# ohjay/snn-modulation-classification

Measured on AMD Instinct MI355X. Metric: IQ windows/sec (RadioML 2x128, T=128), higher is better.
Workload: dtype f32

## Files before the change

### experiments/ablate_c32d.hip

```cpp
#include "../snn_modulation_classification_amd/csrc/dcll_hip.hip"
#include <vector>
int main(int argc, char **argv)
{
    const bool presig = argc > 1 && argv[1][0] == 'p';
    const bool tp = argc > 1 && argv[1][0] == 't';
    const bool co = argc > 1 && !presig && !tp;
    const int B = 1024, T = 128;
    size_t nin = (size_t)T * B * 32 * 8;
    uint32_t *spk_in, *spk_out; float *W, *bias, *tau4, *e0, *e1, *arp, *pv; unsigned long long *dbg;
    hipMalloc(&spk_in, nin * 4); hipMalloc(&spk_out, nin * 4); hipMemset(spk_in, 0x11, nin * 4);
    hipMalloc(&W, 32 * 32 * 49 * 4); hipMalloc(&bias, 128); hipMalloc(&tau4, 512);
    std::vector<float> hw(32 * 32 * 49, 1e-6f), hb(32, 1e-4f), ht(128, 0.9f);
    hipMemcpy(W, hw.data(), hw.size() * 4, hipMemcpyHostToDevice);
    hipMemcpy(bias, hb.data(), 128, hipMemcpyHostToDevice); hipMemcpy(tau4, ht.data(), 512, hipMemcpyHostToDevice);
    size_t ns = (size_t)B * 32 * 256;
    hipMalloc(&e0, ns * 4); hipMalloc(&e1, ns * 4); hipMalloc(&arp, ns * 4);
    hipMemset(e0, 0, ns * 4); hipMemset(e1, 0, ns * 4); hipMemset(arp, 0, ns * 4);
    hipMalloc(&pv, (size_t)T * ns * 4); hipMalloc(&dbg, 4096); hipMemset(dbg, 0, 4096);
    float *dbg_v = nullptr;
    if (presig) hipMalloc(&dbg_v, (size_t)T * ns * 4);
    hipEvent_t a, b; hipEventCreate(&a); hipEventCreate(&b);
    float *pv2 = nullptr, *Wro = nullptr, *ro = nullptr;
    hipStream_t side = nullptr;
    int lo, hi;
    hipDeviceGetStreamPriorityRange(&lo, &hi);
    hipStream_t hot;
    hipStreamCreateWithPriority(&hot, hipStreamNonBlocking, hi);
    if (co) {
        hipMalloc(&pv2, (size_t)T * ns * 4); hipMemset(pv2, 0, (size_t)T * ns * 4);
        hipMalloc(&Wro, 24 * 8192 * 4); hipMemset(Wro, 0, 24 * 8192 * 4); hipMalloc(&ro, (size_t)T * B * 24 * 4);
        hipStreamCreateWithPriority(&side, hipStreamNonBlocking, lo);
    }
    auto launch_side = [&](int n) {
        for (int i = 0; i < n; ++i) dcll_launch_readout_direct(pv2, Wro, nullptr, ro, (long)T * B, 8192, 24, side);
    };
    if (tp) {
        const char *names[3] = {"k_lif_seq_c32rp (row-paired)", "k_lif_seq_c32d (time-paired)", "k_lif_seq_c32d, chain phase only"};
        for (int mode = 0; mode < 3; ++mode) {
            for (int rep = 0; rep < 3 && mode < 2; ++rep) {
                hipMemset(e0, 0, ns * 4); hipMemset(e1, 0, ns * 4); hipMemset(arp, 0, ns * 4);
                hipEventRecord(a);
                if (mode == 0)
                    hipLaunchKernelGGL((k_lif_seq_c32rp<true, 1, 0>), dim3(B), dim3(512), 0, 0, spk_in, dcll_wsrc{W, nullptr, nullptr}, bias, tau4, e0, e1, arp, spk_out, pv, (float *)nullptr, T, B, 0.65f, 1.0f);
                else
                    hipLaunchKernelGGL((k_lif_seq_c32d<true, 1, 0>), dim3(B), dim3(512), 0, 0, spk_in, dcll_wsrc{W, nullptr, nullptr}, bias, tau4, e0, e1, arp, spk_out, pv, (float *)nullptr, T, B, 0.65f, 1.0f);
                hipEventRecord(b); hipEventSynchronize(b);
                float ms; hipEventElapsedTime(&ms, a, b);
                printf("%s B=%d T=%d: %.3f ms\n", names[mode], B, T, ms);
            }
            hipMemset(dbg, 0, 4096);
            if (mode == 0)
                hipLaunchKernelGGL((k_lif_seq_c32rp<true, 1, 1>), dim3(B), dim3(512), 0, 0, spk_in, dcll_wsrc{W, nullptr, nullptr}, bias, tau4, e0, e1, arp, spk_out, pv, (float *)dbg, T, B, 0.65f, 1.0f);
            else if (mode == 1)
                hipLaunchKernelGGL((k_lif_seq_c32d<true, 1, 1>), dim3(B), dim3(512), 0, 0, spk_in, dcll_wsrc{W, nullptr, nullptr}, bias, tau4, e0, e1, arp, spk_out, pv, (float *)dbg, T, B, 0.65f, 1.0f);
            else
                hipLaunchKernelGGL((k_lif_seq_c32d<true, 1, 9>), dim3(B), dim3(512), 0, 0, spk_in, dcll_wsrc{W, nullptr, nullptr}, bias, tau4, e0, e1, arp, spk_out, pv, (float *)dbg, T, B, 0.65f, 1.0f);
            hipDeviceSynchronize();
            unsigned long long h4[64];
            hipMemcpy(h4, dbg, 512, hipMemcpyDeviceToHost);
            const double nst4 = 4.0 * T + 8;
            printf("%s: cycles per stage | non-MFMA phase | barrier 2 | chains + slot write | barrier 1\n", names[mode]);
            for (int w = 0; w < 8; ++w)
                printf("  w%d: %8.0f | %7.0f | %7.0f | %7.0f | %7.0f\n", w, h4[w * 8] / nst4, h4[w * 8 + 1] / nst4, h4[w * 8 + 2] / nst4,
                       h4[w * 8 + 3] / nst4, h4[w * 8 + 4] / nst4);
        }
        return 0;
    }
    if (presig) {
        for (int mode = 0; mode < 2; ++mode) {
            float best = 1e30f;
            for (int rep = 0; rep < 4; ++rep) {
                hipEventRecord(a);
                if (mode == 0)
                    hipLaunchKernelGGL((k_lif_seq_c32rp<true, 1, 0>), dim3(B), dim3(512), 0, 0, spk_in, dcll_wsrc{W, nullptr, nullptr}, bias, tau4, e0, e1, arp, spk_out, pv, (float *)nullptr, T, B, 0.65f, 1.0f);
                else
                    hipLaunchKernelGGL((k_lif_seq_c32rp<true, 2, 0>), dim3(B), dim3(512), 0, 0, spk_in, dcll_wsrc{W, nullptr, nullptr}, bias, tau4, e0, e1, arp, spk_out, (float *)nullptr, pv, T, B, 0.65f, 1.0f);
                hipEventRecord(b); hipEventSynchronize(b);
                float ms; hipEventElapsedTime(&ms, a, b);
                if (ms < best) best = ms;
            }
            printf("k_lif_seq_c32rp B=%d T=%d, buffer = %s: %.3f ms (best of 4)\n", B, T, mode ? "v (pv_presigmoid)" : "sigmoid(v)", best);
            if (mode == 0)
                hipLaunchKernelGGL((k_lif_seq_c32rp<true, 3, 1>), dim3(B), dim3(512), 0, 0, spk_in, dcll_wsrc{W, nullptr, nullptr}, bias, tau4, e0, e1, arp, spk_out, pv, (float *)dbg_v, T, B, 0.65f, 1.0f);
            else
                hipLaunchKernelGGL((k_lif_seq_c32rp<true, 2, 1>), dim3(B), dim3(512), 0, 0, spk_in, dcll_wsrc{W, nullptr, nullptr}, bias, tau4, e0, e1, arp, spk_out, (float *)nullptr, (float *)dbg_v, T, B, 0.65f, 1.0f);
            hipDeviceSynchronize();
            unsigned long long h3[64];
            hipMemcpy(h3, dbg_v, 512, hipMemcpyDeviceToHost);
            const double nst3 = 4.0 * T + 8;
            printf("  cycles per stage | non-MFMA phase | barrier 2 | chains + slot write | barrier 1%s\n", mode ? "" : "   (this variant also stores v: OUT = 3)");
            for (int w = 0; w < 8; ++w)
                printf("  w%d: %8.0f | %7.0f | %7.0f | %7.0f | %7.0f\n", w, h3[w * 8] / nst3, h3[w * 8 + 1] / nst3, h3[w * 8 + 2] / nst3,
                       h3[w * 8 + 3] / nst3, h3[w * 8 + 4] / nst3);
        }
        return 0;
    }
    for (int rep = 0; rep < 3 && !co; ++rep) {
        hipEventRecord(a);
        hipLaunchKernelGGL((k_lif_seq_c32rp<true, 1, 0>), dim3(B), dim3(512), 0, 0, spk_in, dcll_wsrc{W, nullptr, nullptr}, bias, tau4, e0, e1, arp, spk_out, pv, (float *)nullptr, T, B, 0.65f, 1.0f);
        hipEventRecord(b); hipEventSynchronize(b);
        float ms; hipEventElapsedTime(&ms, a, b);
        printf("k_lif_seq_c32rp B=%d T=%d: %.2f ms (ideal at 157.3 TF: %.2f)\n", B, T, ms, 2.0 * 32 * 1568 * 256 * (double)T * B / 157.3e12 * 1e3);
    }
    if (!co) {
        for (int rep = 0; rep < 3; ++rep) {
            hipEventRecord(a);
            hipLaunchKernelGGL((k_lif_seq_c32rp<true, 1, 2>), dim3(B), dim3(512), 0, 0, spk_in, dcll_wsrc{W, nullptr, nullptr}, bias, tau4, e0, e1, arp, spk_out, pv, (float *)nullptr, T, B, 0.65f, 1.0f);
            hipEventRecord(b); hipEventSynchronize(b);
            float ms; hipEventElapsedTime(&ms, a, b);
            printf("k_lif_seq_c32rp, conflict-free B reads (wrong data): %.2f ms\n", ms);
        }
        hipLaunchKernelGGL((k_lif_seq_c32rp<true, 1, 3>), dim3(B), dim3(512), 0, 0, spk_in, dcll_wsrc{W, nullptr, nullptr}, bias, tau4, e0, e1, arp, spk_out, pv, (float *)dbg, T, B, 0.65f, 1.0f);
        unsigned long long h2[64];
        hipMemcpy(h2, dbg, 512, hipMemcpyDeviceToHost);
        const double nst2 = 4.0 * T + 8;
        printf("conflict-free variant: cycles per stage | non-MFMA phase | barrier 2 | chains + slot write | barrier 1\n");
        for (int w = 0; w < 8; ++w)
            printf("  w%d: %8.0f | %7.0f | %7.0f | %7.0f | %7.0f\n", w, h2[w * 8] / nst2, h2[w * 8 + 1] / nst2, h2[w * 8 + 2] / nst2,
                   h2[w * 8 + 3] / nst2, h2[w * 8 + 4] / nst2);
        hipMemset(dbg, 0, 4096);
    }
    if (co) {
        hipDeviceSynchronize();
        launch_side(40);
        hipEventRecord(a, hot);
    }
    hipLaunchKernelGGL((k_lif_seq_c32rp<true, 1, 1>), dim3(B), dim3(512), 0, hot, spk_in, dcll_wsrc{W, nullptr, nullptr}, bias, tau4, e0, e1, arp, spk_out, pv, (float *)dbg, T, B, 0.65f, 1.0f);
    if (co) {
        hipEventRecord(b, hot); hipEventSynchronize(b);
        float ms; hipEventElapsedTime(&ms, a, b);
        printf("k_lif_seq_c32rp B=%d T=%d with the co-resident readout running: %.2f ms\n", B, T, ms);
    }
    hipDeviceSynchronize();
    unsigned long long h[64];
    hipMemcpy(h, dbg, 512, hipMemcpyDeviceToHost);
    const double nst = 4.0 * T + 8;
    printf("wave: cycles per stage | non-MFMA phase | barrier 2 | chains + slot write | barrier 1   (s_memtime ticks per stage)\n");
    for (int w = 0; w < 8; ++w)
        printf("  w%d: %8.0f | %7.0f | %7.0f | %7.0f | %7.0f\n", w, h[w * 8] / nst, h[w * 8 + 1] / nst, h[w * 8 + 2] / nst,
               h[w * 8 + 3] / nst, h[w * 8 + 4] / nst);
    return 0;
}
```

### snn_modulation_classification_amd/csrc/dcll_hip.hip

```cpp
#include "dcll_internal.h"

static thread_local char g_err[DCLL_ERR_LEN] = "";
char *dcll_err_buf(void) { return g_err; }

extern "C" int dcll_version(void) { return DCLL_ABI_VERSION; }
extern "C" const char *dcll_last_error(void) { return g_err; }

constexpr size_t DCLL_TRACE_LEN = 1 << 16;
static thread_local bool g_trace_on = false;
static thread_local size_t g_trace_len = 0;
static thread_local char *g_trace = nullptr;
void dcll_trace_note(const char *name)
{
    if (!g_trace_on || !g_trace) return;
    const size_t n = strlen(name);
    if (g_trace_len + n + 5 >= DCLL_TRACE_LEN) {
        if (g_trace_len + 4 < DCLL_TRACE_LEN && (g_trace_len < 4 || memcmp(g_trace + g_trace_len - 4, "...\n", 4) != 0)) {
            memcpy(g_trace + g_trace_len, "...\n", 4);
            g_trace_len += 4;
        }
        return;
    }
    memcpy(g_trace + g_trace_len, name, n);
    g_trace[g_trace_len + n] = '\n';
    g_trace_len += n + 1;
}
extern "C" int dcll_kernel_trace(int32_t enable)
{
    if (enable) {
        if (!g_trace) g_trace = (char *)malloc(DCLL_TRACE_LEN);
        if (!g_trace) return fail(DCLL_ERR_INVALID, "dcll_kernel_trace: out of host memory");
        g_trace_len = 0;
    }
    g_trace_on = enable != 0;
    return DCLL_OK;
}
extern "C" int64_t dcll_kernel_trace_read(char *buf, int64_t cap)
{
    if (buf && cap > 0) {
        const size_t n = g_trace_len < (size_t)(cap - 1) ? g_trace_len : (size_t)(cap - 1);
        if (n) memcpy(buf, g_trace, n);
        buf[n] = 0;
    }
    return (int64_t)g_trace_len + 1;
}

static inline int split16_max_batch(void)
{
    const char *e = getenv("DCLL_SPLIT16_MAX_BATCH");
    return e && *e ? atoi(e) : 256;
}


extern "C" int dcll_conv_out_shape(const dcll_conv_desc *d, int32_t *ch, int32_t *cw, int32_t *ph, int32_t *pw)
{
    int rc = check_desc(d);
    if (rc) return rc;
    int a, b, c, e;
    conv_shape(d, &a, &b, &c, &e);
    if (ch) *ch = a;
    if (cw) *cw = b;
    if (ph) *ph = c;
    if (pw) *pw = e;
    return DCLL_OK;
}

__global__ void k_trace(const float *__restrict__ x, const float *__restrict__ alpha, const float *__restrict__ tau_m,
                        const float *__restrict__ alphas, const float *__restrict__ tau_s, float *__restrict__ eps0,
                        float *__restrict__ eps1, long n, long per_sample, int tau_is_tensor)
{
    long i = (long)blockIdx.x * blockDim.x + threadIdx.x;
    long stride = (long)gridDim.x * blockDim.x;
    for (; i < n; i += stride) {
        long q = tau_is_tensor ? (i % per_sample) : 0;
        float e0 = eps0[i], e1 = eps1[i];
        trace_update(x[i], alpha[q], tau_m[q], alphas[q], tau_s[q], e0, e1);
        eps0[i] = e0;
        eps1[i] = e1;
    }
}

__global__ void k_conv_lif(dcll_conv_desc d, int ch, int cw, const float *__restrict__ eps1,
                           const dcll_wsrc W, const float *__restrict__ bias, float *__restrict__ arp,
                           float *__restrict__ s_full, float *__restrict__ pv_full, float *__restrict__ v_out, long n)
{
    long i = (long)blockIdx.x * blockDim.x + threadIdx.x;
    if (i >= n) return;
    int xx = (int)(i % cw);
    long r = i / cw;
    int y = (int)(r % ch);
    r /= ch;
    int co = (int)(r % d.c_out);
    long b = r / d.c_out;
    const int cig = d.c_in / d.groups, grp = co / (d.c_out / d.groups);
    const float *e = eps1 + (b * d.c_in + (long)grp * cig) * d.h * d.w;
    const long wbase = (long)co * cig * d.kh * d.kw;
    float acc = bias ? bias[co] : 0.0f;
    const int npair = (cig + 1) >> 1;
    for (int cp = 0; cp < npair; ++cp)
        for (int ky = 0; ky < d.kh; ++ky) {
            int yy = y * d.stride + ky * d.dilation - d.pad_h;
            bool yin = yy >= 0 && yy < d.h;
            for (int kx = 0; kx < d.kw; ++kx) {
                int xq = xx * d.stride + kx * d.dilation - d.pad_w;
                bool in = yin && xq >= 0 && xq < d.w;
#pragma unroll
                for (int hh = 0; hh < 2; ++hh) {
                    int ci = 2 * cp + hh;
                    if (ci < cig) {
                        float ev = in ? e[((long)ci * d.h + yy) * d.w + xq] : 0.0f;
                        acc = __builtin_fmaf(ev, W.at(wbase + ((long)ci * d.kh + ky) * d.kw + kx, co), acc);
                    }
                }
            }
        }
    float v = acc;
    bool s;
    if (d.refractory) {
        float a = arp[i];
        v = refractory(acc, a, d.alpharp, d.wrp, s);
        arp[i] = a;
    } else {
        s = v > 0.0f;
    }
    if (v_out) v_out[i] = v;
    s_full[i] = s ? 1.0f : 0.0f;
    pv_full[i] = sigmoidf_dev(v);
}

template <int KH, int KW, int COG>
__global__ __launch_bounds__(256) void k_conv_lif_tiled(dcll_conv_desc d, int ch, int cw, const float *__restrict__ eps1,
                                                         const dcll_wsrc W, const float *__restrict__ bias,
                                                         float *__restrict__ arp, float *__restrict__ s_full,
                                                         float *__restrict__ pv_full, float *__restrict__ v_out)
{
    constexpr int IH = 16 + KH - 1, IW = 16 + KW - 1, KK = KH * KW;
    __shared__ float in[2][IH * IW];
    __shared__ __attribute__((aligned(16))) float wl[COG * KK * 2];
    const int ntx = (cw + 15) >> 4;
    const int tx0 = (blockIdx.x % ntx) * 16, ty0 = (blockIdx.x / ntx) * 16;
    const int co0 = blockIdx.y * COG;
    const long b = blockIdx.z;
    const int tid = threadIdx.x, lx = tid & 15, ly = tid >> 4;
    const int oy = ty0 + ly, ox = tx0 + lx;
    float acc[COG];
#pragma unroll
    for (int c = 0; c < COG; ++c) acc[c] = (bias && co0 + c < d.c_out) ? bias[co0 + c] : 0.0f;
    const float *eb = eps1 + b * d.c_in * d.h * d.w;
    const int npair = (d.c_in + 1) >> 1;
    for (int cp = 0; cp < npair; ++cp) {
        __syncthreads();
        for (int i = tid; i < 2 * IH * IW; i += 256) {
            const int hh = i / (IH * IW), r = i % (IH * IW);
            const int yy = ty0 + r / IW - d.pad_h, xx = tx0 + r % IW - d.pad_w, ci = 2 * cp + hh;
            const bool ok = ci < d.c_in && yy >= 0 && yy < d.h && xx >= 0 && xx < d.w;
            in[hh][r] = ok ? eb[((long)ci * d.h + yy) * d.w + xx] : 0.0f;
        }
        for (int i = tid; i < COG * KK * 2; i += 256) {
            const int hh = i & 1, tap = (i >> 1) % KK, c = (i >> 1) / KK, ci = 2 * cp + hh;
            wl[i] = (co0 + c < d.c_out && ci < d.c_in) ? W.at(((long)(co0 + c) * d.c_in + ci) * KK + tap, co0 + c) : 0.0f;
        }
        __syncthreads();
        float win[2][KK];
#pragma unroll
        for (int ky = 0; ky < KH; ++ky)
#pragma unroll
            for (int kx = 0; kx < KW; ++kx) {
                win[0][ky * KW + kx] = in[0][(ly + ky) * IW + lx + kx];
                win[1][ky * KW + kx] = in[1][(ly + ky) * IW + lx + kx];
            }
#pragma unroll
        for (int c = 0; c < COG; ++c) {
            const f32x2 *wp = (const f32x2 *)(wl + c * KK * 2);
#pragma unroll
            for (int tap = 0; tap < KK; ++tap) {
                const f32x2 w2 = wp[tap];
                acc[c] = __builtin_fmaf(win[0][tap], w2[0], acc[c]);
                acc[c] = __builtin_fmaf(win[1][tap], w2[1], acc[c]);
            }
        }
    }
    if (oy < ch && ox < cw) {
#pragma unroll
        for (int c = 0; c < COG; ++c) {
            if (co0 + c < d.c_out) {
                const long i = ((b * d.c_out + co0 + c) * ch + oy) * cw + ox;
                float v = acc[c];
                bool s;
                if (d.refractory) {
                    float a = arp[i];
                    v = refractory(acc[c], a, d.alpharp, d.wrp, s);
                    arp[i] = a;
                } else {
                    s = v > 0.0f;
                }
                if (v_out) v_out[i] = v;
                s_full[i] = s ? 1.0f : 0.0f;
                pv_full[i] = sigmoidf_dev(v);
            }
        }
    }
}

__global__ void k_pool(dcll_conv_desc d, int ch, int cw, int ph, int pw, const float *__restrict__ s_full,
                       const float *__restrict__ pv_full, float *__restrict__ s_out, float *__restrict__ pv_out, long n)
{
    long i = (long)blockIdx.x * blockDim.x + threadIdx.x;
    if (i >= n) return;
    int px = (int)(i % pw);
    long r = i / pw;
    int py = (int)(r % ph);
    long bc = r / ph;
    const float *sp = s_full + bc * ch * cw, *pp = pv_full + bc * ch * cw;
    float ms = -INFINITY, mp = -INFINITY;
    int y0 = py * d.pool_h - (d.pool_h - 1) / 2, x0 = px * d.pool_w - (d.pool_w - 1) / 2;
    for (int dy = 0; dy < d.pool_h; ++dy)
        for (int dx = 0; dx < d.pool_w; ++dx) {
            int yy = y0 + dy, xq = x0 + dx;
            if (yy < 0 || yy >= ch || xq < 0 || xq >= cw) continue;
            ms = fmaxf(ms, sp[yy * cw + xq]);
            mp = fmaxf(mp, pp[yy * cw + xq]);
        }
    s_out[i] = ms;
    pv_out[i] = mp;
}

__global__ void k_bwd_dv(dcll_conv_desc d, int ch, int cw, int ph, int pw, const float *__restrict__ v,
                         const float *__restrict__ g_p, const float *__restrict__ g_pv, const float *__restrict__ g_v,
                         const float *__restrict__ i2o_W, float *__restrict__ gvf, long n)
{
    long i = (long)blockIdx.x * blockDim.x + threadIdx.x;
    if (i >= n) return;
    int x = (int)(i % cw);
    long r = i / cw;
    int y = (int)(r % ch);
    r /= ch;
    int co = (int)(r % d.c_out);
    long b = r / d.c_out;
    const int pph = (d.pool_h - 1) / 2, ppw = (d.pool_w - 1) / 2;
    const int py = (y + pph) / d.pool_h, px = (x + ppw) / d.pool_w;
    float g = 0.0f;
    const float pv = sigmoidf_dev(v[i]);
    if (py < ph && px < pw) {
        const float *vp = v + (b * d.c_out + co) * (long)ch * cw;
        const int y0 = py * d.pool_h - pph, x0 = px * d.pool_w - ppw;
        bool is_max = true;
        for (int dy = 0; dy < d.pool_h && is_max; ++dy)
            for (int dx = 0; dx < d.pool_w; ++dx) {
                int yy = y0 + dy, xx = x0 + dx;
                if (yy < 0 || yy >= ch || xx < 0 || xx >= cw || (yy == y && xx == x)) continue;
                float q = sigmoidf_dev(vp[yy * cw + xx]);
                bool before = (yy < y) || (yy == y && xx < x);
                if (q > pv || (before && q == pv)) { is_max = false; break; }
            }
        if (is_max) {
            const long pidx = ((b * d.c_out + co) * ph + py) * pw + px;
            if (g_pv) g = g_pv[pidx];
            if (g_p) {
                const int K = d.c_out * ph * pw;
                const int k = (co * ph + py) * pw + px;
                float acc = 0.0f;
                for (int nn = 0; nn < d.target; ++nn) acc = __builtin_fmaf(g_p[b * d.target + nn], i2o_W[(long)nn * K + k], acc);
                g += acc;
            }
        }
    }
    float out = g * pv * (1.0f - pv);
    if (g_v) out += g_v[i];
    gvf[i] = out;
}

constexpr int WG_MAXTAPS = 64;
__global__ __launch_bounds__(256) void k_bwd_wgrad(dcll_conv_desc d, int ch, int cw, const float *__restrict__ gvf,
                                                    const float *__restrict__ eps1, float *__restrict__ part, int B,
                                                    int RB)
{
    extern __shared__ float sm[];
    const int cig = d.c_in / d.groups;
    const int co = blockIdx.x / cig, cil = blockIdx.x % cig, ci = (co / (d.c_out / d.groups)) * cig + cil;
    const int WP = d.w + 2 * d.pad_w, ntap = d.kh * d.kw;
    const int band = (RB - 1) * d.stride + (d.kh - 1) * d.dilation + 1;
    float *e = sm;
    float *red = sm + band * WP;
    float acc[WG_MAXTAPS];
#pragma unroll
    for (int t = 0; t < WG_MAXTAPS; ++t) acc[t] = 0.0f;
    float accb = 0.0f;
    const long rowlen = (long)cig * ntap + 1;
    float *prow = part + ((long)blockIdx.y * d.c_out + co) * rowlen;
    for (int b = blockIdx.y; b < B; b += gridDim.y) {
        const float *ep = eps1 + ((long)b * d.c_in + ci) * d.h * d.w;
        const float *gp = gvf + ((long)b * d.c_out + co) * ch * cw;
        for (int y0 = 0; y0 < ch; y0 += RB) {
            const int rows = min(RB, ch - y0);
            __syncthreads();
            for (int i = threadIdx.x; i < ((rows - 1) * d.stride + (d.kh - 1) * d.dilation + 1) * WP; i += 256) {
                const int iy = y0 * d.stride + i / WP - d.pad_h, ix = i % WP - d.pad_w;
                e[i] = ((unsigned)iy < (unsigned)d.h && (unsigned)ix < (unsigned)d.w) ? ep[iy * d.w + ix] : 0.0f;
            }
            __syncthreads();
            for (int pos = threadIdx.x; pos < rows * cw; pos += 256) {
                const int yy = pos / cw, xx = pos % cw;
                const float g = gp[(y0 + yy) * cw + xx];
// ... 1039 lines not shown
            auto tapval = [&](int cp, int off) -> float { return (BASES == 2 && cp) ? lds[i1 + off] : lds[i0 + cp * 2 * CHF + off]; };
            float bq[2][7];
#pragma unroll
            for (int kx = 0; kx < 7; ++kx) bq[0][kx] = tapval(0, kx);
#pragma unroll
            for (int r = 0; r < 14; ++r) {
                if (r + 1 < 14) {
                    const int cpn = (r + 1) / 7, kyn = (r + 1) % 7;
#pragma unroll
                    for (int kx = 0; kx < 7; ++kx) bq[(r + 1) & 1][kx] = tapval(cpn, kyn * ROWF + kx);
                }
                __builtin_amdgcn_sched_barrier(0);
#pragma unroll
                for (int kx = 0; kx < 7; ++kx)
                    acc = __builtin_amdgcn_mfma_f32_32x32x2f32(wf[r / 7][(r % 7) * 7 + kx], bq[r & 1][kx], acc, 0, 0, 0);
                __builtin_amdgcn_sched_barrier(0);
            }
            f32x4 *dp = (f32x4 *)(slots + (w * 2 + (g & 1)) * SLOT_FLOATS) + lane;
            if (ABLATE & 4) {
                if (acc[0] + acc[5] + acc[10] + acc[15] == 12345.678f) dp[0] = f32x4{acc[0], acc[1], acc[2], acc[3]};
            } else {
#pragma unroll
                for (int c = 0; c < 4; ++c) {
                    f32x4 v4 = {acc[4 * c + 0], acc[4 * c + 1], acc[4 * c + 2], acc[4 * c + 3]};
                    dp[c * 64] = v4;
                }
            }
        }
        if (loaded && (PRIO & 4)) __builtin_amdgcn_s_setprio(0);
        if (ABLATE & 8) {
            asm volatile("s_waitcnt vmcnt(0) lgkmcnt(0)" ::: "memory");
            unsigned long long x_ = __builtin_amdgcn_s_memtime();
            dbg_mf += x_ - dbg_a;
            __syncthreads();
            dbg_wait += __builtin_amdgcn_s_memtime() - x_;
        } else {
            __syncthreads();
        }
    }
    if ((ABLATE & 8) && lane == 0 && b == 0) {
        unsigned long long tot = __builtin_amdgcn_s_memtime() - dbg_t0;
        unsigned long long *dp = (unsigned long long *)v_out + w * 8;
        dp[0] = tot; dp[1] = dbg_wait; dp[2] = dbg_epi; dp[3] = dbg_tr; dp[4] = dbg_mf;
    }

    const float *fin = lds + ((T - 1) & 1) * IMG_FLOATS;
#pragma unroll
    for (int i = 0; i < 16; ++i) {
        long gidx = (b * 32 + 4 * w + (i >> 2)) * 256 + (i & 3) * 64 + lane;
        eps0_g[gidx] = e0[i];
        eps1_g[gidx] = fin[ioff + (i >> 2) * CHF + (i & 3) * 4 * ROWF];
    }
    if (REFRACTORY) {
#pragma unroll
        for (int k = 0; k < 4; ++k)
#pragma unroll
            for (int rr = 0; rr < 4; ++rr)
                arp_g[(b * 32 + rr + 8 * wq + 4 * h) * 256 + 32 * (2 * k + wpar) + j] = arp[k][rr];
    }
}

template <bool REFRACTORY, int OUT, int DBG = 0>
__global__ __launch_bounds__(512) void k_lif_seq_c32rp(const uint32_t *__restrict__ spk_in, const dcll_wsrc W,
                                                       const float *__restrict__ bias, const float *__restrict__ tau4,
                                                       float *__restrict__ eps0_g, float *__restrict__ eps1_g,
                                                       float *__restrict__ arp_g, uint32_t *__restrict__ spk_out,
                                                       float *__restrict__ pv_out, float *__restrict__ v_out, int T,
                                                       int B, float alpharp, float wrp)
{
    __shared__ __attribute__((aligned(16))) float lds[2 * IMG_FLOATS + (NWAVE * 2 + 1) * SLOT_FLOATS];
    float *slots = lds + 2 * IMG_FLOATS;
    float *sbias = slots + NWAVE * 2 * SLOT_FLOATS;
    const int tid = threadIdx.x, lane = tid & 63, h = lane >> 5, j = lane & 31;
    const int wi = __builtin_amdgcn_readfirstlane(tid >> 6);
    const int w = (DBG & 4) ? wi : ((wi & 1) | ((wi & 4) >> 1) | ((wi & 2) << 1));
    const int wq = w & 3, wpar = w >> 2;
    const long b = blockIdx.x;
    __builtin_amdgcn_s_setprio(3);

    for (int i = tid; i < 2 * IMG_FLOATS; i += 512) lds[i] = 0.0f;
    for (int i = tid; i < SLOT_FLOATS; i += 512) sbias[i] = bias[(i & 3) + 8 * (i >> 8) + 4 * ((i >> 7) & 1)];

    float wf[2][49];
    load_wf_c32(W, j, w, h, wf);

    float e0[4][4];
    const int ioff = (4 * w) * CHF + ((lane >> 4) + 3) * ROWF + (lane & 15) + 3;
    const unsigned long long *in_wave = (const unsigned long long *)(spk_in + (b * 32 + 4 * w) * 8);
    const long in_step = (long)B * 32 * 4;
    __syncthreads();

#pragma unroll
    for (int grp = 0; grp < 4; ++grp) {
        const int c = (grp - w) & 3;
        const float ta = tau4[0 * 32 + 4 * w + c], tm = tau4[1 * 32 + 4 * w + c];
        const float tas = tau4[2 * 32 + 4 * w + c], ts = tau4[3 * 32 + 4 * w + c];
#pragma unroll
        for (int ii = 0; ii < 4; ++ii) {
            const long gidx = (b * 32 + 4 * w + c) * 256 + ii * 64 + lane;
            e0[grp][ii] = eps0_g[gidx];
            float e1 = eps1_g[gidx];
            float xin = (float)((in_wave[c * 4 + ii] >> lane) & 1ull);
            trace_update(xin, ta, tm, tas, ts, e0[grp][ii], e1);
            lds[ioff + c * CHF + ii * 4 * ROWF] = e1;
        }
    }
    float arp[4][4];
#pragma unroll
    for (int k = 0; k < 4; ++k)
#pragma unroll
        for (int rr = 0; rr < 4; ++rr)
            arp[k][rr] = REFRACTORY ? arp_g[(b * 32 + rr + 8 * wq + 4 * h) * 256 + 32 * (2 * k + wpar) + j] : 0.0f;

    const int bbase = (4 * w + h) * CHF + (j >> 4) * ((DBG & 2) ? 16 : ROWF) + (j & 15);
    const unsigned eoff = 4u * (4 * h * 256 + 32 * wpar + j);
#pragma unroll
    for (int k = 0; k < 4; ++k)
#pragma unroll
        for (int rr = 0; rr < 4; ++rr) asm volatile("" ::"v"(arp[k][rr]));
#pragma unroll
    for (int grp = 0; grp < 4; ++grp)
#pragma unroll
        for (int ii = 0; ii < 4; ++ii) asm volatile("" ::"v"(e0[grp][ii]));
#pragma unroll
    for (int cp = 0; cp < 2; ++cp)
#pragma unroll
        for (int k = 0; k < 49; ++k) asm volatile("" ::"v"(wf[cp][k]));
    __syncthreads();

    unsigned long long dbg[4] = {0, 0, 0, 0}, dbg_t0 = 0;
    if (DBG & 1) dbg_t0 = __builtin_amdgcn_s_memtime();
    float sv[4] = {0.f, 0.f, 0.f, 0.f}, ta = 0.f, tm = 0.f, tas = 0.f, ts = 0.f;
    unsigned long long wm[4] = {0, 0, 0, 0};
    auto fetch_trace_inputs = [&](const int g) {
        const int q = g - w;
        if (q >= 0 && q < 4 * T && (q >> 2) + 1 < T) {
            const int p = q & 3, t = q >> 2;
            const float *src = lds + (t & 1) * IMG_FLOATS + ioff + p * CHF;
#pragma unroll
            for (int i = 0; i < 4; ++i) sv[i] = src[i * 4 * ROWF];
            const unsigned long long *ip = in_wave + (long)(t + 1) * in_step + p * 4;
#pragma unroll
            for (int i = 0; i < 4; ++i) wm[i] = ip[i];
            ta = tau4[0 * 32 + 4 * w + p]; tm = tau4[1 * 32 + 4 * w + p];
            tas = tau4[2 * 32 + 4 * w + p]; ts = tau4[3 * 32 + 4 * w + p];
        }
    };
    fetch_trace_inputs(0);
    auto stage = [&](const int g, auto UC) {
        constexpr int U = decltype(UC)::value;
        unsigned long long st0 = 0, st1 = 0, st2 = 0, st3 = 0;
        if (DBG & 1) st0 = __builtin_amdgcn_s_memtime();
        const int q = g - w;
        const bool active = q >= 0 && q < 4 * T;
        const int p = q & 3, t = q >> 2;
        f32x16 accA, accB;
        if (active) {
            const float *inA = (w == 0) ? sbias : slots + ((w - 1) * 2) * SLOT_FLOATS;
            const float *inB = (w == 0) ? sbias : slots + ((w - 1) * 2 + 1) * SLOT_FLOATS;
            const f32x4 *spa = (const f32x4 *)inA + lane, *spb = (const f32x4 *)inB + lane;
#pragma unroll
            for (int c = 0; c < 4; ++c) {
                f32x4 va = spa[c * 64], vb = spb[c * 64];
                accA[4 * c + 0] = va[0]; accA[4 * c + 1] = va[1]; accA[4 * c + 2] = va[2]; accA[4 * c + 3] = va[3];
                accB[4 * c + 0] = vb[0]; accB[4 * c + 1] = vb[1]; accB[4 * c + 2] = vb[2]; accB[4 * c + 3] = vb[3];
            }
        }
        const int qe = g - 8;
        const bool epi = qe >= 0 && qe < 4 * T;
        f32x4 v4 = {0.f, 0.f, 0.f, 0.f};
        if (epi) v4 = *((const f32x4 *)(slots + (7 * 2 + wpar) * SLOT_FLOATS) + wq * 64 + lane);
        const bool tr = active && t + 1 < T;
        const int i0 = (t & 1) * IMG_FLOATS + bbase + p * 4 * ROWF;
        const bool skip = !(DBG & 4);
        const int rl = (skip && p == 0) ? 2 : 0;
        lds_cfloat *ib0 = (lds_cfloat *)(lds + i0), *ib1 = (lds_cfloat *)(lds + i0 + 2 * CHF);
        asm volatile("" : "+v"(ib0), "+v"(ib1));
        float bq[2][7];
        if (active) {
#pragma unroll
            for (int kx = 0; kx < 7; ++kx) bq[0][kx] = ib0[rl * ROWF + kx];
        }
        if (tr) {
            float *dst = lds + ((t + 1) & 1) * IMG_FLOATS + ioff + p * CHF;
#pragma unroll
            for (int i = 0; i < 4; ++i) {
                float a;
                asm("v_cndmask_b32 %0, 0, %1, %2" : "=v"(a) : "v"(ts), "s"(wm[i]));
                const float bb = tas * e0[U][i];
                e0[U][i] = a + bb;
                const float cc = ta * sv[i];
                const float dd = e0[U][i] * tm;
                dst[i * 4 * ROWF] = cc + dd;
            }
        }
        if (epi) {
            const int te = qe >> 2, me = 2 * U + wpar;
            const long ubase = (((long)te * B + b) * 32 + 8 * wq) * 256;
            const auto prs = tile_rsrc(pv_out + ubase), vrs = tile_rsrc(v_out + ubase);
            uint32_t myword = 0;
#pragma unroll
            for (int rr = 0; rr < 4; ++rr) {
                float v = v4[rr];
                bool s;
                if (REFRACTORY) v = refractory(v4[rr], arp[U][rr], alpharp, wrp, s);
                else s = v > 0.0f;
                const unsigned long long mk = __ballot(s);
                const uint32_t mine = h ? (uint32_t)(mk >> 32) : (uint32_t)mk;
                myword = (j == rr) ? mine : myword;
                if (OUT & 1) __builtin_amdgcn_raw_buffer_store_b32(__float_as_uint(sigmoidf_dev(v)), prs, eoff + 4u * (rr * 256 + 64 * U), 0, 0);
                if (OUT & 2) __builtin_amdgcn_raw_buffer_store_b32(__float_as_uint(v), vrs, eoff + 4u * (rr * 256 + 64 * U), 0, 0);
            }
            if (spk_out && j < 4)
                __builtin_amdgcn_raw_buffer_store_b32(myword, tile_rsrc(spk_out + (ubase >> 5)), 4u * ((4 * h + j) * 8 + wpar) + 8u * U, 0, 0);
        }
        if (DBG & 1) { asm volatile("s_waitcnt lgkmcnt(0)" ::: "memory"); st1 = __builtin_amdgcn_s_memtime(); }
        lds_barrier();
        if (DBG & 1) st2 = __builtin_amdgcn_s_memtime();
        fetch_trace_inputs(g + 1);
        if (active) {
            auto chains = [&](auto RLC, auto RHC) {
                constexpr int RL = decltype(RLC)::value, RH = decltype(RHC)::value, NRH = RH - RL, NR = 2 * NRH;
#pragma unroll
                for (int r = 0; r < NR; ++r) {
                    const int cp = r / NRH, rho = RL + r % NRH;
                    if (r + 1 < NR) {
                        const int cpn = (r + 1) / NRH, rhon = RL + (r + 1) % NRH;
#pragma unroll
                        for (int kx = 0; kx < 7; ++kx) bq[(r + 1) & 1][kx] = (cpn ? ib1 : ib0)[rhon * ROWF + kx];
                    }
                    __builtin_amdgcn_sched_barrier(0);
#pragma unroll
                    for (int kx = 0; kx < 7; ++kx) {
                        if (rho <= 6)
                            accA = __builtin_amdgcn_mfma_f32_32x32x2f32(wf[cp][rho * 7 + kx], bq[r & 1][kx], accA, 0, 0, 0);
                        if (rho >= 2)
                            accB = __builtin_amdgcn_mfma_f32_32x32x2f32(wf[cp][(rho - 2) * 7 + kx], bq[r & 1][kx], accB, 0, 0, 0);
                    }
                    __builtin_amdgcn_sched_barrier(0);
                    if (cp == 1 && rho == 6 && r + 1 < NR) {
                        f32x4 *dpa = (f32x4 *)(slots + (w * 2) * SLOT_FLOATS) + lane;
#pragma unroll
                        for (int c = 0; c < 4; ++c)
                            dpa[c * 64] = f32x4{accA[4 * c + 0], accA[4 * c + 1], accA[4 * c + 2], accA[4 * c + 3]};
                        __builtin_amdgcn_sched_barrier(0);
                    }
                }
                if (RH == 7) {
                    f32x4 *dpa = (f32x4 *)(slots + (w * 2) * SLOT_FLOATS) + lane;
#pragma unroll
                    for (int c = 0; c < 4; ++c)
                        dpa[c * 64] = f32x4{accA[4 * c + 0], accA[4 * c + 1], accA[4 * c + 2], accA[4 * c + 3]};
                }
            };
            if (skip && p == 0) chains(std::integral_constant<int, 2>{}, std::integral_constant<int, 9>{});
            else if (skip && p == 3) chains(std::integral_constant<int, 0>{}, std::integral_constant<int, 7>{});
            else chains(std::integral_constant<int, 0>{}, std::integral_constant<int, 9>{});
            f32x4 *dp = (f32x4 *)(slots + (w * 2 + 1) * SLOT_FLOATS) + lane;
#pragma unroll
            for (int c = 0; c < 4; ++c)
                dp[c * 64] = f32x4{accB[4 * c + 0], accB[4 * c + 1], accB[4 * c + 2], accB[4 * c + 3]};
        }
        if (DBG & 1) { asm volatile("s_waitcnt lgkmcnt(0)" ::: "memory"); st3 = __builtin_amdgcn_s_memtime(); }
        lds_barrier();
        if (DBG & 1) {
            const unsigned long long st4 = __builtin_amdgcn_s_memtime();
            dbg[0] += st1 - st0; dbg[1] += st2 - st1; dbg[2] += st3 - st2; dbg[3] += st4 - st3;
        }
    };

    const int nstage = 4 * T + 8;
    for (int g = 0; g < nstage; g += 4) {
        stage(g + 0, std::integral_constant<int, 0>{});
        stage(g + 1, std::integral_constant<int, 1>{});
        stage(g + 2, std::integral_constant<int, 2>{});
        stage(g + 3, std::integral_constant<int, 3>{});
    }

    if ((DBG & 1) && lane == 0 && b == 0) {
        unsigned long long *dp = (unsigned long long *)v_out + w * 8;
        dp[0] = __builtin_amdgcn_s_memtime() - dbg_t0;
        dp[1] = dbg[0]; dp[2] = dbg[1]; dp[3] = dbg[2]; dp[4] = dbg[3];
    }
    const float *fin = lds + ((T - 1) & 1) * IMG_FLOATS;
#pragma unroll
    for (int grp = 0; grp < 4; ++grp) {
        const int c = (grp - w) & 3;
#pragma unroll
        for (int ii = 0; ii < 4; ++ii) {
            const long gidx = (b * 32 + 4 * w + c) * 256 + ii * 64 + lane;
            eps0_g[gidx] = e0[grp][ii];
            eps1_g[gidx] = fin[ioff + c * CHF + ii * 4 * ROWF];
        }
    }
    if (REFRACTORY) {
#pragma unroll
        for (int k = 0; k < 4; ++k)
#pragma unroll
            for (int rr = 0; rr < 4; ++rr)
                arp_g[(b * 32 + rr + 8 * wq + 4 * h) * 256 + 32 * (2 * k + wpar) + j] = arp[k][rr];
    }
}

constexpr int TP_IMGP = IMG_FLOATS + 20;
static_assert(TP_IMGP % 32 == 16 && TP_IMGP >= IMG_FLOATS, "image pitch");
constexpr int TP_ROW_A[8] = {0, 1, 4, 6, 12, 13, 8, 10}, TP_ROW_B[8] = {3, 2, 5, 7, 15, 14, 9, 11};
constexpr int tp_lo(int r) { return r - 3 < 0 ? 0 : r - 3; }
constexpr int tp_hi(int r) { return r + 3 > 15 ? 15 : r + 3; }
constexpr int tp_trace_m(int s) { return (s + 3) & 7; }
constexpr bool tp_trace_next(int s) { return s >= 5; }
constexpr bool tp_reads(int s, int rho) { return rho >= tp_lo(TP_ROW_A[s]) && rho <= tp_hi(TP_ROW_B[s]); }
constexpr uint32_t tp_pack(const int (&r)[8])
{
    uint32_t p = 0;
    for (int i = 0; i < 8; ++i) p |= (uint32_t)r[i] << (4 * i);
    return p;
}
constexpr bool tp_schedule_ok()
{
    int seen = 0, mseen = 0;
    for (int s = 0; s < 8; ++s) {
        if (TP_ROW_A[s] >= TP_ROW_B[s]) return false;
        if (tp_lo(TP_ROW_A[s]) > tp_lo(TP_ROW_B[s]) || tp_hi(TP_ROW_A[s]) > tp_hi(TP_ROW_B[s])) return false;
        if (tp_lo(TP_ROW_B[s]) > tp_hi(TP_ROW_A[s]) + 1) return false;
        seen |= (1 << TP_ROW_A[s]) | (1 << TP_ROW_B[s]);
        const int s2 = (s + 2) & 7;
        const int n = tp_hi(TP_ROW_A[s]) - tp_lo(TP_ROW_A[s]) + tp_hi(TP_ROW_B[s]) - tp_lo(TP_ROW_B[s]) + 2;
        const int n2 = tp_hi(TP_ROW_A[s2]) - tp_lo(TP_ROW_A[s2]) + tp_hi(TP_ROW_B[s2]) - tp_lo(TP_ROW_B[s2]) + 2;
        if (n + n2 != 25) return false;
        const int m = tp_trace_m(s);
        mseen |= 1 << m;
        for (int rho = 2 * m; rho < 2 * m + 2; ++rho) {
            if (tp_trace_next(s)) {
                for (int u = s; u < 8; ++u) if (tp_reads(u, rho)) return false;
            } else {
                for (int u = 0; u < s; ++u) if (tp_reads(u, rho)) return false;
                if (rho == tp_lo(TP_ROW_A[s])) return false;
            }
        }
    }
    return seen == 0xffff && mseen == 0xff;
}
static_assert(tp_schedule_ok(), "k_lif_seq_c32d: tile order / rolling trace schedule");

template <bool REFRACTORY, int OUT, int DBG = 0>
__global__ __launch_bounds__(512) void k_lif_seq_c32d(const uint32_t *__restrict__ spk_in, const dcll_wsrc W,
                                                       const float *__restrict__ bias, const float *__restrict__ tau4,
                                                       float *__restrict__ eps0_g, float *__restrict__ eps1_g,
                                                       float *__restrict__ arp_g, uint32_t *__restrict__ spk_out,
                                                       float *__restrict__ pv_out, float *__restrict__ v_out, int T,
                                                       int B, float alpharp, float wrp)
{
    __shared__ __attribute__((aligned(16))) float lds[2 * TP_IMGP + (NWAVE * 2 + 1) * SLOT_FLOATS];
    float *slots = lds + 2 * TP_IMGP;
    float *sbias = slots + NWAVE * 2 * SLOT_FLOATS;
    const int tid = threadIdx.x, lane = tid & 63, h = lane >> 5, j = lane & 31, px = lane & 15, rb = (lane >> 4) & 1;
    const int wi = __builtin_amdgcn_readfirstlane(tid >> 6);
    const int w = (wi & 1) | ((wi & 4) >> 1) | ((wi & 2) << 1);
    const int wq = w & 3, wpar = w >> 2;
    const long b = blockIdx.x;
    const int NP = T >> 1;
    __builtin_amdgcn_s_setprio(3);

    for (int i = tid; i < 2 * TP_IMGP; i += 512) lds[i] = 0.0f;
    for (int i = tid; i < SLOT_FLOATS; i += 512) sbias[i] = bias[(i & 3) + 8 * (i >> 8) + 4 * ((i >> 7) & 1)];

    float wf[2][49];
    load_wf_c32(W, j, w, h, wf);

    float e0[8][2];
    const int toff = (4 * w + h) * CHF + (rb + 3) * ROWF + px + 3;
    float ta[2], tm[2], tas[2], ts[2];
#pragma unroll
    for (int e = 0; e < 2; ++e) {
        ta[e] = tau4[0 * 32 + 4 * w + 2 * e + h]; tm[e] = tau4[1 * 32 + 4 * w + 2 * e + h];
        tas[e] = tau4[2 * 32 + 4 * w + 2 * e + h]; ts[e] = tau4[3 * 32 + 4 * w + 2 * e + h];
    }
    const uint32_t *in_wave = spk_in + (b * 32 + 4 * w) * 8;
    const long in_step = (long)B * 32 * 8;
    auto in_mask = [&](long t, int e, int m) -> unsigned long long {
        const uint32_t *ip = in_wave + t * in_step + 2 * e * 8 + m;
        return (unsigned long long)ip[0] | ((unsigned long long)ip[8] << 32);
    };
    __syncthreads();

    static_for<0, 8>([&](auto SC) {
        constexpr int S = decltype(SC)::value, M = tp_trace_m(S);
#pragma unroll
        for (int e = 0; e < 2; ++e) {
            const long gidx = (b * 32 + 4 * w + 2 * e + h) * 256 + 32 * M + j;
            e0[S][e] = eps0_g[gidx];
            float e1 = eps1_g[gidx];
            float *dst = lds + toff + e * 2 * CHF + 2 * M * ROWF;
            trace_update((float)((in_mask(0, e, M) >> lane) & 1ull), ta[e], tm[e], tas[e], ts[e], e0[S][e], e1);
            dst[0] = e1;
            trace_update((float)((in_mask(1, e, M) >> lane) & 1ull), ta[e], tm[e], tas[e], ts[e], e0[S][e], e1);
            dst[TP_IMGP] = e1;
        }
    });
    const uint32_t rowpk = wpar ? tp_pack(TP_ROW_B) : tp_pack(TP_ROW_A);
    const int ech = 8 * wq + 4 * h + 2 * rb;
    float arp[8][2];
#pragma unroll
    for (int s = 0; s < 8; ++s) {
        const int re = (rowpk >> (4 * ((s + w) & 7))) & 15;
#pragma unroll
        for (int k = 0; k < 2; ++k) arp[s][k] = REFRACTORY ? arp_g[(b * 32 + ech + k) * 256 + re * 16 + px] : 0.0f;
    }

    const int bbase = (4 * w + h) * CHF + (j >> 4) * TP_IMGP + (j & 15);
    const int eslot = (7 * 2 + wpar) * SLOT_FLOATS + (wq * 64 + h * 32 + px) * 4 + 2 * rb;
    const unsigned eoff = 4u * ((4 * h + 2 * rb) * 256 + px);
    const unsigned soff = (unsigned)(px >> 1) * ((unsigned)B * 1024u) + 32u * (4 * h + 2 * rb + (px & 1));
#pragma unroll
    for (int s = 0; s < 8; ++s)
#pragma unroll
        for (int k = 0; k < 2; ++k) asm volatile("" ::"v"(arp[s][k]), "v"(e0[s][k]));
#pragma unroll
    for (int cp = 0; cp < 2; ++cp)
#pragma unroll
        for (int k = 0; k < 49; ++k) asm volatile("" ::"v"(wf[cp][k]));
    __syncthreads();

    unsigned long long dbg[4] = {0, 0, 0, 0}, dbg_t0 = 0;
    if (DBG & 1) dbg_t0 = __builtin_amdgcn_s_memtime();
    float sv[2] = {0.f, 0.f};
    unsigned long long wm[2][2] = {{0, 0}, {0, 0}};
    auto tracing = [&](const int q, const int s) {
        const int P = q >> 3;
        return !(DBG & 8) && q >= 0 && (tp_trace_next(s) ? P + 1 < NP : (P >= 1 && P < NP));
    };
    auto fetch_trace_inputs = [&](const int q, auto SC) {
        constexpr int S = decltype(SC)::value, M = tp_trace_m(S);
        if (tracing(q, S)) {
            const long t2 = 2 * ((q >> 3) + (tp_trace_next(S) ? 1 : 0));
#pragma unroll
            for (int e = 0; e < 2; ++e) {
                sv[e] = lds[TP_IMGP + toff + e * 2 * CHF + 2 * M * ROWF];
                wm[e][0] = in_mask(t2, e, M);
                wm[e][1] = in_mask(t2 + 1, e, M);
            }
        }
    };
    auto stage = [&](const int g, auto SC) {
        constexpr int S = decltype(SC)::value, RA = TP_ROW_A[S], RB = TP_ROW_B[S];
        constexpr int LO = tp_lo(RA), HI = tp_hi(RB), NRH = HI - LO + 1, NR = 2 * NRH;
        unsigned long long st0 = 0, st1 = 0, st2 = 0, st3 = 0;
        if (DBG & 1) st0 = __builtin_amdgcn_s_memtime();
        const int q = g - w;
        const bool active = q >= 0 && q < 8 * NP;
        f32x16 accA, accB;
        if (active) {
            const float *inA = (w == 0) ? sbias : slots + ((w - 1) * 2) * SLOT_FLOATS;
            const float *inB = (w == 0) ? sbias : slots + ((w - 1) * 2 + 1) * SLOT_FLOATS;
            const f32x4 *spa = (const f32x4 *)inA + lane, *spb = (const f32x4 *)inB + lane;
#pragma unroll
            for (int c = 0; c < 4; ++c) {
                f32x4 va = spa[c * 64], vb = spb[c * 64];
                accA[4 * c + 0] = va[0]; accA[4 * c + 1] = va[1]; accA[4 * c + 2] = va[2]; accA[4 * c + 3] = va[3];
                accB[4 * c + 0] = vb[0]; accB[4 * c + 1] = vb[1]; accB[4 * c + 2] = vb[2]; accB[4 * c + 3] = vb[3];
            }
        }
        const int qe = g - 8;
        const bool epi = !(DBG & 8) && qe >= 0 && qe < 8 * NP;
        f32x2 v0 = {0.f, 0.f}, v1 = {0.f, 0.f};
        if (epi) {
            v0 = *(const f32x2 *)(slots + eslot);
            v1 = *(const f32x2 *)(slots + eslot + 64);
        }
        lds_cfloat *ib0 = (lds_cfloat *)(lds + bbase + (LO + 3) * ROWF), *ib1 = (lds_cfloat *)(lds + bbase + (LO + 3) * ROWF + 2 * CHF);
        asm volatile("" : "+v"(ib0), "+v"(ib1));
        float bq[2][7];
        if (active) {
#pragma unroll
            for (int kx = 0; kx < 7; ++kx) bq[0][kx] = ib0[kx];
        }
        if (tracing(q, S)) {
            float *dst = lds + toff + 2 * tp_trace_m(S) * ROWF;
#pragma unroll
            for (int e = 0; e < 2; ++e) {
                float e1 = sv[e];
#pragma unroll
                for (int dt = 0; dt < 2; ++dt) {
                    float a;
                    asm("v_cndmask_b32 %0, 0, %1, %2" : "=v"(a) : "v"(ts[e]), "s"(wm[e][dt]));
                    const float bb = tas[e] * e0[S][e];
                    e0[S][e] = a + bb;
                    const float cc = ta[e] * e1;
                    const float dd = e0[S][e] * tm[e];
                    e1 = cc + dd;
                    dst[e * 2 * CHF + dt * TP_IMGP] = e1;
                }
            }
        }
        if (epi) {
            const int te = 2 * (qe >> 3);
            const int re = (rowpk >> (4 * (g & 7))) & 15;
            const long ubase = (((long)te * B + b) * 32 + 8 * wq) * 256, ustep = (long)B * 32 * 256;
            float vv[2][2];
            unsigned long long mk[2][2];
#pragma unroll
            for (int k = 0; k < 2; ++k) {
                bool s0, s1;
                if (REFRACTORY) {
                    vv[k][0] = refractory(v0[k], arp[S][k], alpharp, wrp, s0);
                    vv[k][1] = refractory(v1[k], arp[S][k], alpharp, wrp, s1);
                } else {
                    vv[k][0] = v0[k]; vv[k][1] = v1[k];
                    s0 = v0[k] > 0.0f; s1 = v1[k] > 0.0f;
                }
                mk[k][0] = __ballot(s0); mk[k][1] = __ballot(s1);
            }
#pragma unroll
            for (int dt = 0; dt < 2; ++dt) {
                const auto prs = tile_rsrc(pv_out + ubase + dt * ustep), vrs = tile_rsrc(v_out + ubase + dt * ustep);
#pragma unroll
                for (int k = 0; k < 2; ++k) {
                    if (OUT & 1) __builtin_amdgcn_raw_buffer_store_b32(__float_as_uint(sigmoidf_dev(vv[k][dt])), prs, eoff + 4u * (k * 256), re * 64, 0);
                    if (OUT & 2) __builtin_amdgcn_raw_buffer_store_b32(__float_as_uint(vv[k][dt]), vrs, eoff + 4u * (k * 256), re * 64, 0);
                }
            }
            if (spk_out) {
                uint32_t myword = 0;
#pragma unroll
                for (int dt = 0; dt < 2; ++dt)
#pragma unroll
                    for (int k = 0; k < 2; ++k) {
                        const uint32_t mine = h ? (uint32_t)(mk[k][dt] >> 32) : (uint32_t)mk[k][dt];
                        myword = (px == k + 2 * dt) ? mine : myword;
                    }
                myword >>= 16 * rb;
                if (px < 4)
                    __builtin_amdgcn_raw_buffer_store_b16((unsigned short)myword, tile_rsrc(spk_out + (ubase >> 5)), soff, 4 * (re >> 1) + 2 * (re & 1), 0);
            }
        }
        if (DBG & 1) { asm volatile("s_waitcnt lgkmcnt(0)" ::: "memory"); st1 = __builtin_amdgcn_s_memtime(); }
        lds_barrier();
        if (DBG & 1) st2 = __builtin_amdgcn_s_memtime();
        fetch_trace_inputs(q + 1, std::integral_constant<int, (S + 1) & 7>{});
        if (active) {
#pragma unroll
            for (int r = 0; r < NR; ++r) {
                const int cp = r / NRH, rho = LO + r % NRH;
                if (r + 1 < NR) {
                    const int cpn = (r + 1) / NRH, rhon = (r + 1) % NRH;
#pragma unroll
                    for (int kx = 0; kx < 7; ++kx) bq[(r + 1) & 1][kx] = (cpn ? ib1 : ib0)[rhon * ROWF + kx];
                }
                __builtin_amdgcn_sched_barrier(0);
#pragma unroll
                for (int kx = 0; kx < 7; ++kx) {
                    if (rho >= tp_lo(RA) && rho <= tp_hi(RA))
                        accA = __builtin_amdgcn_mfma_f32_32x32x2f32(wf[cp][(rho - RA + 3) * 7 + kx], bq[r & 1][kx], accA, 0, 0, 0);
                    if (rho >= tp_lo(RB) && rho <= tp_hi(RB))
                        accB = __builtin_amdgcn_mfma_f32_32x32x2f32(wf[cp][(rho - RB + 3) * 7 + kx], bq[r & 1][kx], accB, 0, 0, 0);
                }
                __builtin_amdgcn_sched_barrier(0);
                if (cp == 1 && rho == tp_hi(RA)) {
                    f32x4 *dpa = (f32x4 *)(slots + (w * 2) * SLOT_FLOATS) + lane;
#pragma unroll
                    for (int c = 0; c < 4; ++c)
                        dpa[c * 64] = f32x4{accA[4 * c + 0], accA[4 * c + 1], accA[4 * c + 2], accA[4 * c + 3]};
                    __builtin_amdgcn_sched_barrier(0);
                }
            }
            f32x4 *dp = (f32x4 *)(slots + (w * 2 + 1) * SLOT_FLOATS) + lane;
#pragma unroll
            for (int c = 0; c < 4; ++c)
                dp[c * 64] = f32x4{accB[4 * c + 0], accB[4 * c + 1], accB[4 * c + 2], accB[4 * c + 3]};
        }
        if (DBG & 1) { asm volatile("s_waitcnt lgkmcnt(0)" ::: "memory"); st3 = __builtin_amdgcn_s_memtime(); }
        lds_barrier();
        if (DBG & 1) {
            const unsigned long long st4 = __builtin_amdgcn_s_memtime();
            dbg[0] += st1 - st0; dbg[1] += st2 - st1; dbg[2] += st3 - st2; dbg[3] += st4 - st3;
        }
    };

    const int nstage = 8 * NP + 8;
    for (int g = 0; g < nstage; ++g) {
        switch ((g - w) & 7) {
        case 0: stage(g, std::integral_constant<int, 0>{}); break;
        case 1: stage(g, std::integral_constant<int, 1>{}); break;
        case 2: stage(g, std::integral_constant<int, 2>{}); break;
        case 3: stage(g, std::integral_constant<int, 3>{}); break;
        case 4: stage(g, std::integral_constant<int, 4>{}); break;
        case 5: stage(g, std::integral_constant<int, 5>{}); break;
        case 6: stage(g, std::integral_constant<int, 6>{}); break;
        default: stage(g, std::integral_constant<int, 7>{}); break;
        }
    }

    if ((DBG & 1) && lane == 0 && b == 0) {
        unsigned long long *dp = (unsigned long long *)v_out + w * 8;
        dp[0] = __builtin_amdgcn_s_memtime() - dbg_t0;
        dp[1] = dbg[0]; dp[2] = dbg[1]; dp[3] = dbg[2]; dp[4] = dbg[3];
    }
    static_for<0, 8>([&](auto SC) {
        constexpr int S = decltype(SC)::value, M = tp_trace_m(S);
#pragma unroll
        for (int e = 0; e < 2; ++e) {
            const long gidx = (b * 32 + 4 * w + 2 * e + h) * 256 + 32 * M + j;
            eps0_g[gidx] = e0[S][e];
            eps1_g[gidx] = lds[TP_IMGP + toff + e * 2 * CHF + 2 * M * ROWF];
        }
    });
    if (REFRACTORY) {
#pragma unroll
        for (int s = 0; s < 8; ++s) {
            const int re = (rowpk >> (4 * ((s + w) & 7))) & 15;
#pragma unroll
            for (int k = 0; k < 2; ++k) arp_g[(b * 32 + ech + k) * 256 + re * 16 + px] = arp[s][k];
        }
    }
}

__global__ void k_permute_readout(const float *__restrict__ Wt, float *__restrict__ Wp, int N)
{
    int i = blockIdx.x * blockDim.x + threadIdx.x;
    if (i >= N * 8192) return;
    int rr = i & 3, lane = (i >> 2) & 63;
    int r = i >> 8;
    int n = r % N;
    r /= N;
    int wq = r & 3, me = r >> 2;
    int co = rr + 8 * wq + 4 * (lane >> 5), pix = 32 * me + (lane & 31);
    Wp[i] = Wt[(long)n * 8192 + co * 256 + pix];
}

static inline unsigned nblk(long n, int bs) { return (unsigned)((n + bs - 1) / bs); }

static int launch_readout(const float *pv, const float *Wt, const float *bias, float *out, long rows, int K, int N,
                          hipStream_t st, int mode = DCLL_READOUT_AUTO)
{
    if (rows == 0 || N == 0) return DCLL_OK;
    const bool fast = (K % RO_KC == 0) && N <= 64 && (((uintptr_t)pv | (uintptr_t)Wt) & 15) == 0 &&
                      K < (1 << 22);
    const bool direct_ok = fast && K % 64 == 0 && N <= 48 && K <= 16384 && mode != DCLL_READOUT_LDS;
    if (direct_ok && mode == DCLL_READOUT_CORESIDENT)
        return dcll_launch_readout_direct(pv, Wt, bias, out, rows, K, N, st);
    if (fast && mode == DCLL_READOUT_T16) return dcll_launch_readout_t16(pv, Wt, bias, out, rows, K, N, 0, st);
    const char *form = "k_readout";
    if (rows <= 2048) {
        form = "k_readout_rows";
        hipLaunchKernelGGL(k_readout_rows, dim3((unsigned)((rows + RS_RB - 1) / RS_RB), (N + RS_NG - 1) / RS_NG), dim3(256),
                           0, st, pv, Wt, bias, out, rows, K, N);
    } else if (fast && K % RK_KC == 0 && K >= 65536 && rows < 256L * RO_ROWS) {
        form = "k_readout_ks";
        if (N <= 32)
            hipLaunchKernelGGL(k_readout_ks<1>, dim3(nblk(rows, RK_ROWS)), dim3(256), 0, st, pv, Wt, bias, out, rows, K, N, 0);
        else
            hipLaunchKernelGGL(k_readout_ks<2>, dim3(nblk(rows, RK_ROWS)), dim3(256), 0, st, pv, Wt, bias, out, rows, K, N, 0);
    } else if (fast && mode != DCLL_READOUT_LDS) {
        return dcll_launch_readout_t16(pv, Wt, bias, out, rows, K, N, 0, st);
    } else if (fast && N <= 32) {
        form = "k_readout_v4";
        hipLaunchKernelGGL(k_readout_v4<1>, dim3(nblk(rows, RO_ROWS)), dim3(256), 0, st, pv, Wt, bias, out, rows, K, N);
    } else if (fast) {
        form = "k_readout_v4";
        hipLaunchKernelGGL(k_readout_v4<2>, dim3(nblk(rows, RO_ROWS)), dim3(256), 0, st, pv, Wt, bias, out, rows, K, N);
    } else {
        dim3 grid(nblk(rows, RO_ROWS), (N + 31) / 32);
        hipLaunchKernelGGL(k_readout, grid, dim3(256), 0, st, pv, Wt, bias, out, rows, K, N);
    }
    HIP_CHECK_LAUNCH(form);
    return DCLL_OK;
}

extern "C" int dcll_readout(const float *pv, const float *Wt, const float *bias, float *out, int64_t rows, int32_t K,
                            int32_t N, void *stream)
{
    if (rows == 0) return DCLL_OK;
    if (!pv || !Wt || !out || rows < 0 || K < 1 || N < 1) return fail(DCLL_ERR_INVALID, "dcll_readout: bad argument");
    return launch_readout(pv, Wt, bias, out, rows, K, N, (hipStream_t)stream);
}

extern "C" int dcll_readout_mode(const float *pv, const float *Wt, const float *bias, float *out, int64_t rows,
                                 int32_t K, int32_t N, int32_t mode, void *stream)
{
    if (rows == 0) return DCLL_OK;
    if (!pv || !Wt || !out || rows < 0 || K < 1 || N < 1 || mode < DCLL_READOUT_AUTO || mode > DCLL_READOUT_T16)
        return fail(DCLL_ERR_INVALID, "dcll_readout_mode: bad argument");
    return launch_readout(pv, Wt, bias, out, rows, K, N, (hipStream_t)stream, mode);
}

__global__ __launch_bounds__(256) void k_readout_sum(const float *__restrict__ part, const float *__restrict__ bias,
                                                      float *__restrict__ out, long n_out, int N, int nslice)
{
    __shared__ float red[4][64];
    const long i = (long)blockIdx.x * 64 + (threadIdx.x & 63);
    const int grp = threadIdx.x >> 6;
    float acc = 0.0f;
    if (i < n_out) {
        const int per = (nslice + 3) / 4, s0 = grp * per, s1 = min(nslice, s0 + per);
        for (int sl = s0; sl < s1; ++sl) acc += part[(long)sl * n_out + i];
    }
    red[grp][threadIdx.x & 63] = acc;
    __syncthreads();
    if (grp == 0 && i < n_out) {
        const int l = threadIdx.x & 63;
        out[i] = (bias ? bias[i % N] : 0.0f) + (((red[0][l] + red[1][l]) + red[2][l]) + red[3][l]);
    }
}

static int splitk_slice(int64_t rows, int32_t K, int32_t N)
{
    if (rows < 1 || N < 1 || N > 64) return 0;
    if (K >= 65536 && K % 4096 == 0) {
        return rows <= 2048 ? 4096 : K / 8;
    }
    if (rows <= 2048 && K >= 2048 && K < 65536 && K % 256 == 0) return (rows <= 512 && N <= 32) ? 128 : 256;
    return 0;
}

extern "C" int64_t dcll_readout_splitk_scratch(int64_t rows, int32_t K, int32_t N)
{
    const int ks = splitk_slice(rows, K, N);
    return ks ? (int64_t)(K / ks) * rows * N : 0;
}

extern "C" int dcll_readout_splitk(const float *pv, const float *Wt, const float *bias, float *out, float *scratch,
                                   int64_t scratch_floats, int64_t rows, int32_t K, int32_t N, void *stream)
{
    if (rows == 0 || N == 0) return DCLL_OK;
    if (!pv || !Wt || !out || !scratch || rows < 0 || K < 1 || N < 1)
        return fail(DCLL_ERR_INVALID, "dcll_readout_splitk: bad argument");
    const int ks = splitk_slice(rows, K, N);
    if (ks == 0 || ((((uintptr_t)pv | (uintptr_t)Wt)) & 15) != 0)
        return fail(DCLL_ERR_UNSUPPORTED, "dcll_readout_splitk: needs N <= 64, 16-byte aligned operands and K >= 65536 with "
                                          "K % 4096 == 0, or rows <= 2048 with 2048 <= K < 65536, K % 256 == 0");
    if (scratch_floats < dcll_readout_splitk_scratch(rows, K, N))
        return fail(DCLL_ERR_INVALID, "dcll_readout_splitk: scratch too small (dcll_readout_splitk_scratch)");
    hipStream_t st = (hipStream_t)stream;
    const int nslice = K / ks;
    if (ks != 4096) {
        int rc = dcll_launch_readout_t16(pv, Wt, nullptr, scratch, rows, K, N, ks, st);
        if (rc) return rc;
    } else {
        dim3 grid(nblk(rows, RK_ROWS), nslice);
        if (N <= 32) hipLaunchKernelGGL(k_readout_ks<1>, grid, dim3(256), 0, st, pv, Wt, bias, scratch, rows, K, N, 4096);
        else hipLaunchKernelGGL(k_readout_ks<2>, grid, dim3(256), 0, st, pv, Wt, bias, scratch, rows, K, N, 4096);
        HIP_CHECK_LAUNCH("k_readout_ks (split K)");
    }
    hipLaunchKernelGGL(k_readout_sum, dim3(nblk(rows * N, 64)), dim3(256), 0, st, scratch, bias, out, rows * N, N, nslice);
    HIP_CHECK_LAUNCH("k_readout_sum");
    return DCLL_OK;
}

static int act_nslice(int32_t K)
{
    if (K < 65536 || K % 256 != 0) return 0;
    int n = 8;
    while (n < 64 && K / (2 * n) >= 8192 && K % (2 * n * RO_KC) == 0) n *= 2;
    return n;
}
extern "C" int64_t dcll_readout_act_scratch(int64_t rows, int32_t K, int32_t N)
{
    return (rows > 0 && N > 0) ? (int64_t)act_nslice(K) * rows * N : 0;
}

extern "C" int dcll_readout_act(const float *pv, const float *Wt, const float *bias, float *out, float *scratch,
                                int64_t scratch_floats, int64_t rows, int32_t K, int32_t N, int32_t act, void *stream)
{
    if (rows == 0 || N == 0) return DCLL_OK;
    if (!pv || !Wt || !out || rows < 0 || K < 1 || N < 1 || (act != DCLL_ACT_NONE && act != DCLL_ACT_SIGMOID))
        return fail(DCLL_ERR_INVALID, "dcll_readout_act: bad argument");
    if (!(K % RO_KC == 0 && K < (1 << 22) && N <= 64 && (((uintptr_t)pv | (uintptr_t)Wt) & 15) == 0))
        return fail(DCLL_ERR_UNSUPPORTED, "dcll_readout_act: needs K % 32 == 0, K < 2^22, N <= 64, 16-byte aligned pv / Wt");
    hipStream_t st = (hipStream_t)stream;
    const int64_t need = dcll_readout_act_scratch(rows, K, N);
    if (need == 0) return dcll_launch_readout_t16(pv, Wt, bias, out, rows, K, N, 0, st, act);
    if (!scratch || scratch_floats < need)
        return fail(DCLL_ERR_INVALID, "dcll_readout_act: K >= 65536 is split over K and needs scratch (dcll_readout_act_scratch)");
    const int ns = act_nslice(K);
    int rc = dcll_launch_readout_t16(pv, Wt, nullptr, scratch, rows, K, N, K / ns, st, act);
    if (rc) return rc;
    hipLaunchKernelGGL(k_readout_sum, dim3(nblk(rows * N, 64)), dim3(256), 0, st, scratch, bias, out, rows * N, N, ns);
    HIP_CHECK_LAUNCH("k_readout_sum");
    return DCLL_OK;
}

constexpr int STEP_WLS = 49, STEP_WCH = 64 * STEP_WLS + 4;
__device__ __forceinline__ float buf_ldf(__amdgpu_buffer_rsrc_t rs, unsigned voff, unsigned soff)
{
    return __uint_as_float(__builtin_amdgcn_raw_buffer_load_b32(rs, voff, soff, 0));
}
__device__ __forceinline__ void buf_stf(float v, __amdgpu_buffer_rsrc_t rs, unsigned voff, unsigned soff)
{
    __builtin_amdgcn_raw_buffer_store_b32(__float_as_uint(v), rs, voff, soff, 0);
}
constexpr unsigned BUF_OOB = 0x80000000u;
template <bool Q8>
struct step_wchunk {
    static constexpr int NW = 13;
    int raw[NW];
    float qs[NW];
    unsigned goff[NW];
    int loff[NW];
    __amdgpu_buffer_rsrc_t rs;
    __device__ __forceinline__ void init(int tid, const dcll_wsrc &W)
    {
        constexpr bool q8 = Q8;
        rs = q8 ? tile_rsrc(W.q) : tile_rsrc(W.f);
        int co = tid >= 196 ? 2 : tid >= 98 ? 1 : 0, r = tid - 98 * co;
#pragma unroll
        for (int i = 0; i < NW; ++i) {
            const bool valid = i < NW - 1 || tid < 32 * 98 - 256 * (NW - 1);
            const int cv = valid ? co : 0, rv = valid ? r : 0, hh = rv >= 49 ? 1 : 0;
            goff[i] = (unsigned)(cv * 1568 + rv) * (q8 ? 1u : 4u);
            loff[i] = valid ? (hh * 32 + cv) * STEP_WLS + (rv - 49 * hh) : 64 * STEP_WLS;
            qs[i] = q8 ? W.scale[cv] : 0.0f;
            r += 60;
            co += 2;
            if (r >= 98) { r -= 98; co += 1; }
        }
    }
    __device__ __forceinline__ void fetch(int cp)
    {
        if (Q8) {
#pragma unroll
            for (int i = 0; i < NW; ++i) raw[i] = (int)(int8_t)__builtin_amdgcn_raw_buffer_load_b8(rs, goff[i], (unsigned)cp * 98u, 0);
            return;
        }
#pragma unroll
        for (int i = 0; i < NW; ++i) raw[i] = (int)__builtin_amdgcn_raw_buffer_load_b32(rs, goff[i], (unsigned)cp * 392u, 0);
    }
    __device__ __forceinline__ void store(float *wch, int buf) const
    {
        if (Q8) {
#pragma unroll
            for (int i = 0; i < NW; ++i) wch[buf * STEP_WCH + loff[i]] = (float)raw[i] * qs[i];
            return;
        }
#pragma unroll
        for (int i = 0; i < NW; ++i) wch[buf * STEP_WCH + loff[i]] = __int_as_float(raw[i]);
    }
};

template <bool REFRACTORY, int DBG = 0, bool Q8 = false>
__global__ __launch_bounds__(256) void k_lif_step_c32(const float *__restrict__ x, const dcll_wsrc W,
                                                       const float *__restrict__ bias, const float *__restrict__ alpha,
                                                       const float *__restrict__ tau_m, const float *__restrict__ alphas,
                                                       const float *__restrict__ tau_s, int tau_is_tensor,
                                                       float *__restrict__ eps0_g, float *__restrict__ eps1_g,
                                                       float *__restrict__ arp_g, float *__restrict__ out_s,
                                                       float *__restrict__ out_pv, float *__restrict__ out_v,
                                                       float alpharp, float wrp)
{
    __shared__ __attribute__((aligned(16))) float lds[IMG_FLOATS + 2 * STEP_WCH + 32];
    float *img = lds, *wch = lds + IMG_FLOATS, *sbias = wch + 2 * STEP_WCH;
    const int tid = threadIdx.x, lane = tid & 63, h = lane >> 5, j = lane & 31;
    const int w = __builtin_amdgcn_readfirstlane(tid >> 6);
    const long b = blockIdx.x;
    unsigned long long stamp0 = 0, stamp1 = 0, stamp2 = 0, real0 = 0;
    if (DBG & 32) {
        stamp0 = __builtin_amdgcn_s_memtime();
        real0 = __builtin_amdgcn_s_memrealtime();
    }

    if (tid < 32) sbias[tid] = bias[tid];
    step_wchunk<Q8> wc;
    auto fetch_w = [&](int cp) { wc.fetch(cp); };
    auto store_w = [&](int buf) { wc.store(wch, buf); };
    const auto xrs = tile_rsrc(x + b * 8192), e0rs = tile_rsrc(eps0_g + b * 8192), e1rs = tile_rsrc(eps1_g + b * 8192);
    const auto ars = tile_rsrc(alpha), tmrs = tile_rsrc(tau_m), asrs = tile_rsrc(alphas), tsrs = tile_rsrc(tau_s);
    const unsigned tvo = 4u * tid;
    const unsigned tcv0 = tau_is_tensor ? tvo : 0u, tcv1 = tau_is_tensor ? tvo + 1024u : 0u;
    const unsigned tcs = tau_is_tensor ? 2048u : 0u;
    float tx[2], te0[2], te1[2], ta[2], ttm[2], tas[2], tts[2];
    auto fetch_t = [&](int cp) {
        const unsigned so = 2048u * cp, tso = tcs * cp;
#pragma unroll
        for (int i = 0; i < 2; ++i) {
            if (DBG & 4) {
                tx[i] = te0[i] = te1[i] = (float)tid;
            } else {
                tx[i] = buf_ldf(xrs, tvo + 1024u * i, so);
                te0[i] = buf_ldf(e0rs, tvo + 1024u * i, so);
                te1[i] = buf_ldf(e1rs, tvo + 1024u * i, so);
            }
            const unsigned tv = i ? tcv1 : tcv0;
            ta[i] = buf_ldf(ars, tv, tso);
            ttm[i] = buf_ldf(tmrs, tv, tso);
            tas[i] = buf_ldf(asrs, tv, tso);
            tts[i] = buf_ldf(tsrs, tv, tso);
        }
    };
    const int ipix = ((tid >> 4) + 3) * ROWF + (tid & 15) + 3;
    auto finish_t = [&](int cp) {
        const unsigned so = 2048u * cp;
#pragma unroll
        for (int i = 0; i < 2; ++i) {
            trace_update(tx[i], ta[i], ttm[i], tas[i], tts[i], te0[i], te1[i]);
            if (!(DBG & 4) || te0[i] == 12345.678f) {
                buf_stf(te0[i], e0rs, tvo + 1024u * i, so);
                buf_stf(te1[i], e1rs, tvo + 1024u * i, so);
            }
            img[(2 * cp + i) * CHF + ipix] = te1[i];
        }
    };
    fetch_t(0);
    wc.init(tid, W);
    fetch_w(0);
    const unsigned ovo = 4096u * h + 4u * j, oso = 256u * w;
    const auto aprs = tile_rsrc(arp_g + b * 8192);
    float arp_pre[2][16];
    if (REFRACTORY && !(DBG & 2)) {
#pragma unroll
        for (int tl = 0; tl < 2; ++tl)
#pragma unroll
            for (int r = 0; r < 16; ++r)
                arp_pre[tl][r] = buf_ldf(aprs, ovo + 1024u * (r & 3) + 128u * tl, oso + 8192u * (r >> 2));
    }
    {
        constexpr int NZ4 = IMG_FLOATS / 4, NZF = NZ4 / 256;
        f32x4 *z = (f32x4 *)img + tid;
#pragma unroll
// ... 793 lines not shown
        if (nchunk > njob) nchunk = njob;
        hipLaunchKernelGGL((k_bwd_wgrad_c32<22, 484, true>), dim3((unsigned)nchunk), dim3(512), 0, st, scratch, eps1,
                           part, B, d->h, d->w);
        HIP_CHECK_LAUNCH("k_bwd_wgrad_c32 (tiled)");
    } else {
        const int WP = d->w + 2 * d->pad_w;
        const int rows_fit = (48 * 1024 / 4 - 4 * (WG_MAXTAPS + 1)) / WP;
        int RB = rows_fit < (d->kh - 1) * d->dilation + 1 ? 0 : (rows_fit - (d->kh - 1) * d->dilation - 1) / d->stride + 1;
        if (RB < 1) return fail(DCLL_ERR_UNSUPPORTED, "dcll_conv_lif_backward: input rows too wide for the LDS-staged weight-gradient kernel");
        if (RB > ch) RB = ch;
        const size_t lds = ((size_t)((RB - 1) * d->stride + (d->kh - 1) * d->dilation + 1) * WP + 4 * (WG_MAXTAPS + 1)) * sizeof(float);
        if (nchunk > 64) nchunk = 64;
        if (nchunk > B) nchunk = B;
        hipLaunchKernelGGL(k_bwd_wgrad, dim3(d->c_out * (d->c_in / d->groups), (unsigned)nchunk), dim3(256), lds, st, *d, ch, cw,
                           scratch, eps1, part, B, RB);
        HIP_CHECK_LAUNCH(RB < ch ? "k_bwd_wgrad (row bands)" : "k_bwd_wgrad");
    }
    if (open_part) {
        *open_part = part;
        *open_nchunk = (int32_t)nchunk;
    } else {
        if (nchunk >= 64)
            hipLaunchKernelGGL(k_bwd_reduce4<16>, dim3(nblk(per_chunk, 64)), dim3(1024), 0, st, part, dW, db, (int)nchunk, d->c_out, rowlen);
        else if (nchunk >= 16)
            hipLaunchKernelGGL(k_bwd_reduce4<4>, dim3(nblk(per_chunk, 64)), dim3(256), 0, st, part, dW, db, (int)nchunk, d->c_out, rowlen);
        else
            hipLaunchKernelGGL(k_bwd_reduce, dim3(nblk(per_chunk, 256)), dim3(256), 0, st, part, dW, db, (int)nchunk, d->c_out, rowlen);
        HIP_CHECK_LAUNCH(nchunk >= 64 ? "k_bwd_reduce4<16>" : nchunk >= 16 ? "k_bwd_reduce4<4>" : "k_bwd_reduce");
    }
    if (g_o) {
        const int K = d->c_out * ph * pw, N = d->target;
        float *opart = open_part ? part + nchunk * per_chunk : part;
        long nsplit = (scratch_floats - (opart - scratch)) / ((long)N * (K + 1));
        if (nsplit > 16) nsplit = 16;
        if (nsplit > B) nsplit = B;
        if (N <= 32 && K % 32 == 0) {
            hipLaunchKernelGGL(k_bwd_outgrad_mfma, dim3(K / 32), dim3(256), 0, st, g_o, pv_pooled, d_outW, d_outb, B, N, K);
            HIP_CHECK_LAUNCH("k_bwd_outgrad_mfma");
        } else if (N <= 32 && nsplit >= 1) {
            hipLaunchKernelGGL(k_bwd_outgrad_part, dim3(nblk((long)K + N, 256), (unsigned)nsplit), dim3(256), 0, st, g_o,
                               pv_pooled, opart, B, N, K);
            HIP_CHECK_LAUNCH("k_bwd_outgrad_part");
            hipLaunchKernelGGL(k_bwd_outgrad_reduce, dim3(nblk((long)N * (K + 1), 256)), dim3(256), 0, st, opart, d_outW,
                               d_outb, (int)nsplit, N, K);
            HIP_CHECK_LAUNCH("k_bwd_outgrad_reduce");
        } else {
            hipLaunchKernelGGL(k_bwd_outgrad, dim3(nblk((long)N * (K + 1), 256)), dim3(256), 0, st, g_o, pv_pooled,
                               d_outW, d_outb, B, N, K);
            HIP_CHECK_LAUNCH("k_bwd_outgrad");
        }
    }
    return DCLL_OK;
}

extern "C" int dcll_conv_lif_backward(const dcll_conv_desc *d, const float *eps1, const float *v, const float *pv_pooled,
                                      const float *g_p, const float *g_o, const float *g_pv, const float *g_v,
                                      const float *i2o_W, float *dW, float *db, float *d_outW, float *d_outb,
                                      float *scratch, int64_t scratch_floats, int32_t B, void *stream)
{
    return conv_lif_backward_impl(d, eps1, v, pv_pooled, g_p, g_o, g_pv, g_v, i2o_W, dW, db, d_outW, d_outb, scratch,
                                  scratch_floats, B, stream, nullptr, nullptr);
}

extern "C" int dcll_conv_lif_backward_open(const dcll_conv_desc *d, const float *eps1, const float *v, const float *pv_pooled,
                                           const float *g_p, const float *g_o, const float *g_pv, const float *g_v,
                                           const float *i2o_W, float *d_outW, float *d_outb, float *scratch,
                                           int64_t scratch_floats, int32_t B, const float **part, int32_t *nchunk, void *stream)
{
    if (!part || !nchunk) return fail(DCLL_ERR_INVALID, "dcll_conv_lif_backward_open: null part / nchunk");
    return conv_lif_backward_impl(d, eps1, v, pv_pooled, g_p, g_o, g_pv, g_v, i2o_W, nullptr, nullptr, d_outW, d_outb, scratch,
                                  scratch_floats, B, stream, part, nchunk);
}

extern "C" int dcll_conv_lif_backward_any(const dcll_conv_desc *d, const float *eps1, const float *v, const float *pv_pooled,
                                          const float *g_p, const float *g_o, const float *g_pv, const float *g_v,
                                          const float *i2o_W, float *dW, float *db, float *d_outW, float *d_outb,
                                          float *scratch, int64_t scratch_floats, int32_t B, void *stream)
{
    return conv_lif_backward_impl(d, eps1, v, pv_pooled, g_p, g_o, g_pv, g_v, i2o_W, dW, db, d_outW, d_outb, scratch,
                                  scratch_floats, B, stream, nullptr, nullptr, false, true);
}

extern "C" int dcll_conv_lif_backward_any_open(const dcll_conv_desc *d, const float *eps1, const float *v, const float *pv_pooled,
                                               const float *g_p, const float *g_o, const float *g_pv, const float *g_v,
                                               const float *i2o_W, float *d_outW, float *d_outb, float *scratch,
                                               int64_t scratch_floats, int32_t B, const float **part, int32_t *nchunk, void *stream)
{
    if (!part || !nchunk) return fail(DCLL_ERR_INVALID, "dcll_conv_lif_backward_any_open: null part / nchunk");
    return conv_lif_backward_impl(d, eps1, v, pv_pooled, g_p, g_o, g_pv, g_v, i2o_W, nullptr, nullptr, d_outW, d_outb, scratch,
                                  scratch_floats, B, stream, part, nchunk, false, true);
}

extern "C" int dcll_conv_lif_backward_open_multi(dcll_bwd_item *items, int32_t n, void *stream)
{
    const char *who = "dcll_conv_lif_backward_open_multi";
    if (n == 0) return DCLL_OK;
    if (!items || n < 0 || n > BWD_MULTI_MAX) return fail(DCLL_ERR_INVALID, "1 .. 8 items", who);
    bool joint = n > 1;
    int npc = -1, frompv = -1;
    bwd_dv_items it;
    memset(&it, 0, sizeof(it));
    unsigned gx = 1, gy = 1;
    for (int i = 0; i < n; ++i) {
        const dcll_bwd_item &a = items[i];
        if (a.reserved != 0) return fail(DCLL_ERR_INVALID, "dcll_bwd_item.reserved must be 0", who);
        if (!a.d || !a.eps1 || !a.scratch || a.B < 1) return fail(DCLL_ERR_INVALID, "null pointer / empty batch", who);
        int rc = check_desc(a.d);
        if (rc) return rc;
        const bool nopool = a.d->pool_h == 1 && a.d->pool_w == 1 && a.d->target <= 32;
        if (!a.v && !(nopool && a.pv_pooled))
            return fail(DCLL_ERR_INVALID, "v may be NULL only for a layer without pooling whose pv is given", who);
        if (a.g_p && !a.i2o_W) return fail(DCLL_ERR_INVALID, "g_p needs i2o_W", who);
        int ch, cw, ph, pw;
        conv_shape(a.d, &ch, &cw, &ph, &pw);
        const long Kmap = (long)a.d->c_out * ch * cw;
        if ((long)a.B * Kmap > a.scratch_floats) return fail(DCLL_ERR_INVALID, "scratch too small", who);
        const int cls = a.d->target <= 8 ? 8 : a.d->target <= 16 ? 16 : a.d->target <= 24 ? 24 : 32, fp = a.v ? 0 : 1;
        if (!nopool || Kmap >= (1L << 31) || (npc >= 0 && (cls != npc || fp != frompv))) joint = false;
        npc = cls, frompv = fp;
        if (joint) {
            it.v[i] = a.v ? a.v : a.pv_pooled, it.g_p[i] = a.g_p, it.g_pv[i] = a.g_pv, it.g_v[i] = a.g_v, it.i2o_W[i] = a.i2o_W;
            it.gvf[i] = a.scratch, it.K[i] = (int)Kmap, it.N[i] = a.d->target, it.B[i] = a.B;
            gx = max(gx, (unsigned)nblk(Kmap, 256)), gy = max(gy, (unsigned)nblk(a.B, 16));
        }
    }
    hipStream_t st = (hipStream_t)stream;
    if (joint) {
        const dim3 grid(gx, gy, (unsigned)n);
#define DCLL_DVM(NP_)                                                                                                   \
    do {                                                                                                                \
        if (frompv) hipLaunchKernelGGL((k_bwd_dv_nopool_m<NP_, true>), grid, dim3(256), 0, st, it, 16);                  \
        else hipLaunchKernelGGL((k_bwd_dv_nopool_m<NP_, false>), grid, dim3(256), 0, st, it, 16);                        \
    } while (0)
        if (npc == 8) DCLL_DVM(8);
        else if (npc == 16) DCLL_DVM(16);
        else if (npc == 24) DCLL_DVM(24);
        else DCLL_DVM(32);
#undef DCLL_DVM
        HIP_CHECK_LAUNCH("k_bwd_dv_nopool_m");
    }
    for (int i = 0; i < n; ++i) {
        dcll_bwd_item &a = items[i];
        int rc = conv_lif_backward_impl(a.d, a.eps1, a.v, a.pv_pooled, a.g_p, a.g_o, a.g_pv, a.g_v, a.i2o_W, nullptr, nullptr,
                                        a.d_outW, a.d_outb, a.scratch, a.scratch_floats, a.B, stream, &a.part, &a.nchunk, joint);
        if (rc) return rc;
    }
    return DCLL_OK;
}

template <bool SIG>
__global__ __launch_bounds__(256) void k_pv_lowhigh(const float *__restrict__ pv, long per_step, int iter0,
                                                     float thr_low, float thr_high,
                                                     unsigned long long *__restrict__ counts)
{
    __shared__ unsigned red[2][4];
    const int k = blockIdx.y;
    const long t = ((long)(iter0 / 20) + k + 1) * 20 - iter0 - 1;
    const float *p = pv + t * per_step;
    unsigned lo = 0, hi = 0;
    const long stride = (long)gridDim.x * 256;
    long i = (long)blockIdx.x * 256 + threadIdx.x;
    if ((((uintptr_t)p) & 15) == 0) {
        const long n4 = per_step >> 2;
        for (; i < n4 + stride - 1 - (n4 + stride - 1) % stride; i += stride) {
            f32x4 v = {.5f, .5f, .5f, .5f};
            const bool in = i < n4;
            if (in) v = ((const f32x4 *)p)[i];
#pragma unroll
            for (int e = 0; e < 4; ++e) {
                const float q = SIG ? sigmoidf_dev(v[e]) : v[e];
                lo += __popcll(__ballot(in && q < thr_low));
                hi += __popcll(__ballot(in && q >= thr_high));
            }
        }
        i = n4 * 4 + (long)blockIdx.x * 256 + threadIdx.x;
    }
    for (; i < per_step + stride - 1 - (per_step + stride - 1) % stride; i += stride) {
        const bool in = i < per_step;
        const float v = in ? (SIG ? sigmoidf_dev(p[i]) : p[i]) : 0.5f;
        lo += __popcll(__ballot(in && v < thr_low));
        hi += __popcll(__ballot(in && v >= thr_high));
    }
    const int lane = threadIdx.x & 63, wave = threadIdx.x >> 6;
    if (lane == 0) { red[0][wave] = lo; red[1][wave] = hi; }
    __syncthreads();
    if (threadIdx.x < 2) {
        const unsigned tot = red[threadIdx.x][0] + red[threadIdx.x][1] + red[threadIdx.x][2] + red[threadIdx.x][3];
        if (tot) atomicAdd(counts + 2 * k + threadIdx.x, (unsigned long long)tot);
    }
}

static float f32_ceil(double e)
{
    float f = (float)e;
    if ((double)f < e) f = nextafterf(f, INFINITY);
    return f;
}

static inline int n_sampled_steps(int iter0, int T) { return (iter0 + T) / 20 - iter0 / 20; }

static int launch_pv_lowhigh(const float *pv, long per_step, int T, int iter0, unsigned long long *counts,
                             hipStream_t st, const char *who, bool presig = false)
{
    if (iter0 < 0) return fail(DCLL_ERR_INVALID, "negative iteration count", who);
    const int ns = n_sampled_steps(iter0, T);
    if (ns == 0) return DCLL_OK;
    if (!pv) return fail(DCLL_ERR_INVALID, "pv statistics need the pv output of the call", who);
    if (hipMemsetAsync(counts, 0, (size_t)ns * 2 * sizeof(unsigned long long), st) != hipSuccess) {
        (void)hipGetLastError();
        return fail(DCLL_ERR_LAUNCH, "hipMemsetAsync of the pv counters failed", who);
    }
    const double e1 = 1.0 / 19.0, e18 = 18.0 * (1.0 / 19.0);
    long nb = (per_step / 4 + 255) / 256;
    if (nb < 1) nb = 1;
    if (nb > 1024) nb = 1024;
    if (presig)
        hipLaunchKernelGGL(k_pv_lowhigh<true>, dim3((unsigned)nb, (unsigned)ns), dim3(256), 0, st, pv, per_step, iter0,
                           f32_ceil(e1), f32_ceil(e18), counts);
    else
        hipLaunchKernelGGL(k_pv_lowhigh<false>, dim3((unsigned)nb, (unsigned)ns), dim3(256), 0, st, pv, per_step, iter0,
                           f32_ceil(e1), f32_ceil(e18), counts);
    HIP_CHECK_LAUNCH("k_pv_lowhigh");
    return DCLL_OK;
}

extern "C" int dcll_pv_lowhigh_act(const float *pv, int64_t per_step, int32_t T, int32_t iter0, uint64_t *counts,
                                   int32_t act, void *stream)
{
    if (T < 0 || per_step < 0 || iter0 < 0 || (act != DCLL_ACT_NONE && act != DCLL_ACT_SIGMOID))
        return fail(DCLL_ERR_INVALID, "dcll_pv_lowhigh: bad argument");
    if (T == 0 || per_step == 0 || n_sampled_steps(iter0, T) == 0) return DCLL_OK;
    if (!counts) return fail(DCLL_ERR_INVALID, "dcll_pv_lowhigh: null counters");
    return launch_pv_lowhigh(pv, per_step, T, iter0, (unsigned long long *)counts, (hipStream_t)stream, "dcll_pv_lowhigh",
                             act == DCLL_ACT_SIGMOID);
}

extern "C" int dcll_pv_lowhigh(const float *pv, int64_t per_step, int32_t T, int32_t iter0, uint64_t *counts,
                               void *stream)
{
    return dcll_pv_lowhigh_act(pv, per_step, T, iter0, counts, DCLL_ACT_NONE, stream);
}

extern "C" int32_t dcll_pv_lowhigh_steps(int32_t iter0, int32_t T) { return (iter0 < 0 || T < 0) ? 0 : n_sampled_steps(iter0, T); }

static int check_seq_geometry(const dcll_conv_desc *d, int c_in, const char *who)
{
    int rc = check_desc(d);
    if (rc) return rc;
    const bool small = d->h == 16 && d->w == 16;
    const bool tiled = d->h >= 8 && d->h % 8 == 0 && d->w >= 32 && d->w % 32 == 0;
    if (!plain_conv(d) || d->c_in != c_in || d->c_out > 32 || (c_in == 32 && d->c_out != 32) || !(small || tiled) || d->kh != 7 ||
        d->kw != 7 || d->pad_h != 3 || d->pad_w != 3 || d->pool_h != 1 || d->pool_w != 1)
        return fail(DCLL_ERR_UNSUPPORTED,
                    "sequence kernel supports 7x7 pad 3, pool 1, c_out<=32 (==32 for c_in 32) on a 16x16 plane or a plane "
                    "with h % 8 == 0, w % 32 == 0", who);
    return DCLL_OK;
}

extern "C" int dcll_permute_readout(const float *Wt, float *Wp, int32_t N, void *stream)
{
    if (!Wt || !Wp || N < 1) return fail(DCLL_ERR_INVALID, "dcll_permute_readout: bad argument");
    hipLaunchKernelGGL(k_permute_readout, dim3(nblk((long)N * 8192, 256)), dim3(256), 0, (hipStream_t)stream, Wt, Wp, N);
    HIP_CHECK_LAUNCH("k_permute_readout");
    return DCLL_OK;
}

constexpr int DCLL_C32D_MIN_T = 8;

struct seq_outs { float *pv, *v, *copy_dst; };
static inline seq_outs presig_outs(float *pv_out, float *v_out, bool presig)
{
    if (!presig || !pv_out) return {pv_out, v_out, nullptr};
    if (!v_out) return {nullptr, pv_out, nullptr};
    return {nullptr, v_out, pv_out};
}
static int presig_copy(const seq_outs &o, long n, hipStream_t st, const char *who)
{
    if (!o.copy_dst) return DCLL_OK;
    if (hipMemcpyAsync(o.copy_dst, o.v, (size_t)n * sizeof(float), hipMemcpyDeviceToDevice, st) != hipSuccess) {
        (void)hipGetLastError();
        return fail(DCLL_ERR_LAUNCH, "copy of v into pv_out failed", who);
    }
    return DCLL_OK;
}

template <bool R, int NRO>
static void launch_c32(int out, int B, hipStream_t st, const uint32_t *spk_in, dcll_wsrc W, const float *b,
                       const float *tau4, float *eps0, float *eps1, float *arp, uint32_t *spk_out, float *pv_out,
                       float *v_out, const float *ro_Wp, const float *ro_b, float *ro_out, int T, float alpharp,
                       float wrp)
{
#define DCLL_LAUNCH_C32(O)                                                                                             \
    hipLaunchKernelGGL((k_lif_seq_c32<R, O, NRO>), dim3(B), dim3(512), 0, st, spk_in, W, b, tau4, eps0, eps1, arp,     \
                       spk_out, pv_out, v_out, ro_Wp, ro_b, ro_out, T, B, alpharp, wrp)
    switch (out) {
    case 0: DCLL_LAUNCH_C32(0); break;
    case 1: DCLL_LAUNCH_C32(1); break;
    case 2: DCLL_LAUNCH_C32(2); break;
    default: DCLL_LAUNCH_C32(3); break;
    }
#undef DCLL_LAUNCH_C32
}

static int dcll_conv_lif_sequence_run(const dcll_conv_desc *d, const uint32_t *spk_in, dcll_wsrc W, const float *b,
                                      const float *tau4, float *eps0, float *eps1, float *arp, uint32_t *spk_out,
                                      float *pv_out, float *v_out, const float *ro_Wp, const float *ro_b,
                                      float *ro_out, int32_t n_ro, float *state_scratch, int32_t T, int32_t B,
                                      hipStream_t st)
{
    if (n_ro != 0 && n_ro != 24 && n_ro != 48)
        return fail(DCLL_ERR_UNSUPPORTED, "dcll_conv_lif_sequence: fused readout supports 24 or 48 rows (target 24)");
    if (n_ro && (!ro_Wp || !ro_b || !ro_out)) return fail(DCLL_ERR_INVALID, "dcll_conv_lif_sequence: fused readout needs ro_Wp, ro_b, ro_out");
    const int out = (pv_out ? 1 : 0) | (v_out ? 2 : 0);
    if (d->h != 16 || d->w != 16) {
        if (n_ro) return fail(DCLL_ERR_UNSUPPORTED, "dcll_conv_lif_sequence: fused readout only on the 16x16 plane");
        return dcll_launch_seq_c32t(d, spk_in, W, b, tau4, eps0, eps1, arp, spk_out, pv_out, v_out, state_scratch, T, B, st);
    }
    if (n_ro == 0 && T >= DCLL_C32D_MIN_T) {
        const bool tp = (T & 1) == 0;
#define DCLL_LAUNCH_C32D(K, R, O)                                                                                       \
    hipLaunchKernelGGL((K<R, O>), dim3(B), dim3(512), 0, st, spk_in, W, b, tau4, eps0, eps1, arp, spk_out, pv_out,      \
                       v_out, T, B, d->alpharp, d->wrp)
#define DCLL_LAUNCH_C32D_O(K, R)                                                                                        \
    switch (out) {                                                                                                     \
    case 0: DCLL_LAUNCH_C32D(K, R, 0); break;                                                                          \
    case 1: DCLL_LAUNCH_C32D(K, R, 1); break;                                                                          \
    case 2: DCLL_LAUNCH_C32D(K, R, 2); break;                                                                          \
    default: DCLL_LAUNCH_C32D(K, R, 3); break;                                                                         \
    }
        if (tp) {
            if (d->refractory) { DCLL_LAUNCH_C32D_O(k_lif_seq_c32d, true) } else { DCLL_LAUNCH_C32D_O(k_lif_seq_c32d, false) }
            HIP_CHECK_LAUNCH("k_lif_seq_c32d");
        } else {
            if (d->refractory) { DCLL_LAUNCH_C32D_O(k_lif_seq_c32rp, true) } else { DCLL_LAUNCH_C32D_O(k_lif_seq_c32rp, false) }
            HIP_CHECK_LAUNCH("k_lif_seq_c32rp");
        }
#undef DCLL_LAUNCH_C32D_O
#undef DCLL_LAUNCH_C32D
        return DCLL_OK;
    }
#define DCLL_ARGS out, B, st, spk_in, W, b, tau4, eps0, eps1, arp, spk_out, pv_out, v_out, ro_Wp, ro_b, ro_out, T, d->alpharp, d->wrp
    if (d->refractory) {
        if (n_ro == 0) launch_c32<true, 0>(DCLL_ARGS);
        else if (n_ro == 24) launch_c32<true, 24>(DCLL_ARGS);
        else launch_c32<true, 48>(DCLL_ARGS);
    } else {
        if (n_ro == 0) launch_c32<false, 0>(DCLL_ARGS);
        else if (n_ro == 24) launch_c32<false, 24>(DCLL_ARGS);
        else launch_c32<false, 48>(DCLL_ARGS);
    }
#undef DCLL_ARGS
    HIP_CHECK_LAUNCH("k_lif_seq_c32");
    return DCLL_OK;
}

extern "C" int dcll_conv_lif_sequence(const dcll_conv_desc *d, const uint32_t *spk_in, const float *Wf, const float *b,
                                      const float *tau4, float *eps0, float *eps1, float *arp, uint32_t *spk_out,
                                      float *pv_out, float *v_out, const float *ro_Wp, const float *ro_b,
                                      float *ro_out, int32_t n_ro, float *state_scratch, uint64_t *pv_lowhigh,
                                      int32_t iter0, const dcll_layer_opts *opts, int32_t T, int32_t B, void *stream)
{
    const char *who = "dcll_conv_lif_sequence";
    int rc = check_desc(d);
    if (rc) return rc;
    const bool w3 = dcll_seq_w3_geometry(d) && d->c_in == 64;
    if (!w3) {
        rc = check_seq_geometry(d, 32, who);
        if (rc) return rc;
    }
    if (T == 0 || B == 0) return DCLL_OK;
    rc = check_opts(Wf, opts, true, who);
    if (rc) return rc;
    if (!spk_in || !b || !tau4 || !eps0 || !eps1) return fail(DCLL_ERR_INVALID, "null pointer", who);
    if (d->refractory && !arp) return fail(DCLL_ERR_INVALID, "refractory layer needs arp", who);
    if (T < 0 || B < 0) return fail(DCLL_ERR_INVALID, "negative size", who);
    const bool presig = opts && opts->pv_presigmoid;
    if (presig && n_ro) return fail(DCLL_ERR_INVALID, "pv_presigmoid cannot be combined with the fused readout", who);
    const dcll_wsrc W = make_wsrc(Wf, opts);
    hipStream_t st = (hipStream_t)stream;
    long per_step;
    if (w3) {
        if (n_ro) return fail(DCLL_ERR_UNSUPPORTED, "fused readout only for the 7x7 layers on the 16x16 plane", who);
        rc = dcll_launch_seq_w3(d, spk_in, nullptr, W, b, tau4, eps0, eps1, arp, spk_out, pv_out, v_out, presig, T, B, st);
        per_step = (long)B * d->c_out * d->h * (d->w / 2);
    } else {
        const seq_outs o = presig_outs(pv_out, v_out, presig);
        rc = dcll_conv_lif_sequence_run(d, spk_in, W, b, tau4, eps0, eps1, arp, spk_out, o.pv, o.v, ro_Wp, ro_b, ro_out,
                                        n_ro, state_scratch, T, B, st);
        per_step = (long)B * d->c_out * d->h * d->w;
        if (!rc) rc = presig_copy(o, per_step * T, st, who);
    }
    if (rc || !pv_lowhigh) return rc;
    return launch_pv_lowhigh(pv_out, per_step, T, iter0, (unsigned long long *)pv_lowhigh, st, who, presig);
}

static int launch_c1(const dcll_conv_desc *d, const int32_t *cells, const float *iq, const float *thr_i,
                     const float *thr_q, dcll_iq_tail tail, int L, int t0, dcll_wsrc W, const float *b, const float *tau4, float *eps0,
                     float *eps1, float *arp, uint32_t *spk_out, float *pv_out, float *v_out, float *state_scratch,
                     uint64_t *pv_lowhigh, int iter0, bool presig, int T, int B, hipStream_t st)
{
    const char *who = "dcll_conv_lif_sequence_cells/_iq";
    const long per_step = (long)B * d->c_out * d->h * d->w;
    if (pv_lowhigh) {
        int rc = launch_c1(d, cells, iq, thr_i, thr_q, tail, L, t0, W, b, tau4, eps0, eps1, arp, spk_out, pv_out, v_out,
                           state_scratch, nullptr, 0, presig, T, B, st);
        if (rc) return rc;
        return launch_pv_lowhigh(pv_out, per_step, T, iter0, (unsigned long long *)pv_lowhigh, st, who, presig);
    }
    if (presig && pv_out && v_out) {
        int rc = launch_c1(d, cells, iq, thr_i, thr_q, tail, L, t0, W, b, tau4, eps0, eps1, arp, spk_out, nullptr, v_out,
                           state_scratch, nullptr, 0, false, T, B, st);
        if (rc) return rc;
        return presig_copy(seq_outs{nullptr, v_out, pv_out}, per_step * T, st, who);
    }
    if (d->h != 16 || d->w != 16)
        return dcll_launch_seq_c1t(d, cells, iq, thr_i, thr_q, tail, L, t0, W, b, tau4, eps0, eps1, arp, spk_out, pv_out, v_out,
                                   state_scratch, T, B, st, presig);
    const bool fastpath = d->c_out == 32 && spk_out && pv_out && !v_out;
    if (presig && pv_out && !fastpath) { v_out = pv_out; pv_out = nullptr; }
#define DCLL_LAUNCH_C1(R, F, Q)                                                                                         \
    hipLaunchKernelGGL((k_lif_seq_c1<R, F, Q>), dim3(B), dim3(256), 0, st, d->c_out, cells, iq, thr_i, thr_q, tail, L, t0, W,  \
                       b, tau4, eps0, eps1, arp, spk_out, pv_out, v_out, T, B, d->alpharp, d->wrp)
#define DCLL_LAUNCH_C1Q(R, F)                                                                                           \
    do { if (iq) DCLL_LAUNCH_C1(R, F, true); else DCLL_LAUNCH_C1(R, F, false); } while (0)
    if (d->refractory) {
        if (fastpath && presig) DCLL_LAUNCH_C1Q(true, 2);
        else if (fastpath) DCLL_LAUNCH_C1Q(true, 1);
        else DCLL_LAUNCH_C1Q(true, 0);
    } else {
        if (fastpath && presig) DCLL_LAUNCH_C1Q(false, 2);
        else if (fastpath) DCLL_LAUNCH_C1Q(false, 1);
        else DCLL_LAUNCH_C1Q(false, 0);
    }
#undef DCLL_LAUNCH_C1Q
#undef DCLL_LAUNCH_C1
    HIP_CHECK_LAUNCH("k_lif_seq_c1");
    return DCLL_OK;
}

extern "C" int dcll_conv_lif_sequence_cells(const dcll_conv_desc *d, const int32_t *cells, const float *Wf, const float *b,
                                            const float *tau4, float *eps0, float *eps1, float *arp, uint32_t *spk_out,
                                            float *pv_out, float *v_out, float *state_scratch, uint64_t *pv_lowhigh,
                                            int32_t iter0, const dcll_layer_opts *opts, int32_t T, int32_t B, void *stream)
{
    const char *who = "dcll_conv_lif_sequence_cells";
    int rc = check_desc(d);
    if (rc) return rc;
    const bool w3 = dcll_seq_w3_geometry(d) && d->c_in == 1;
    if (!w3) {
        rc = check_seq_geometry(d, 1, who);
        if (rc) return rc;
    }
    if (T == 0 || B == 0) return DCLL_OK;
    rc = check_opts(Wf, opts, true, who);
    if (rc) return rc;
    if (!cells || !b || !tau4 || !eps0 || !eps1) return fail(DCLL_ERR_INVALID, "null pointer", who);
    if (d->refractory && !arp) return fail(DCLL_ERR_INVALID, "refractory layer needs arp", who);
    if (T < 0 || B < 0) return fail(DCLL_ERR_INVALID, "negative size", who);
    const bool presig = opts && opts->pv_presigmoid;
    const dcll_wsrc W = make_wsrc(Wf, opts);
    if (w3) {
        rc = dcll_launch_seq_w3(d, nullptr, cells, W, b, tau4, eps0, eps1, arp, spk_out, pv_out, v_out, presig, T, B,
                                (hipStream_t)stream);
        if (rc || !pv_lowhigh) return rc;
        return launch_pv_lowhigh(pv_out, (long)B * d->c_out * d->h * (d->w / 2), T, iter0, (unsigned long long *)pv_lowhigh,
                                 (hipStream_t)stream, who, presig);
    }
    return launch_c1(d, cells, nullptr, nullptr, nullptr, make_iq_tail(nullptr), 0, 0, W, b, tau4, eps0, eps1, arp, spk_out, pv_out, v_out,
                     state_scratch, pv_lowhigh, iter0, presig, T, B, (hipStream_t)stream);
}

extern "C" int dcll_conv_lif_sequence_iq(const dcll_conv_desc *d, const float *iq, const float *thr_i, const float *thr_q,
                                         const dcll_iq_tail *tail, int32_t L, int32_t t0, const float *Wf, const float *b, const float *tau4,
                                         float *eps0, float *eps1, float *arp, uint32_t *spk_out, float *pv_out,
                                         float *v_out, float *state_scratch, uint64_t *pv_lowhigh, int32_t iter0,
                                         const dcll_layer_opts *opts, int32_t T, int32_t B, void *stream)
{
    const char *who = "dcll_conv_lif_sequence_iq";
    int rc = check_seq_geometry(d, 1, who);
    if (rc) return rc;
    if (T == 0 || B == 0) return DCLL_OK;
    rc = check_opts(Wf, opts, true, who);
    if (rc) return rc;
    if (!iq || !thr_i || !thr_q || !b || !tau4 || !eps0 || !eps1) return fail(DCLL_ERR_INVALID, "null pointer", who);
    if (tail && tail->tail_mask && (!tail->thr_i_tail || !tail->thr_q_tail)) return fail(DCLL_ERR_INVALID, "tail mask without tail tables", who);
    if (d->refractory && !arp) return fail(DCLL_ERR_INVALID, "refractory layer needs arp", who);
    if (T < 0 || B < 0 || t0 < 0 || t0 + T > L) return fail(DCLL_ERR_INVALID, "window [t0, t0+T) outside the IQ row", who);
    if (T > C1_MAXT) return fail(DCLL_ERR_UNSUPPORTED, "at most 4096 timesteps per launch", who);
    return launch_c1(d, nullptr, iq, thr_i, thr_q, make_iq_tail(tail), L, t0, make_wsrc(Wf, opts), b, tau4, eps0, eps1, arp, spk_out, pv_out,
                     v_out, state_scratch, pv_lowhigh, iter0, opts && opts->pv_presigmoid, T, B, (hipStream_t)stream);
}

extern "C" int dcll_argmax_vote(const float *logits, int32_t *clout, int32_t *vote, int32_t T, int32_t B, int32_t N,
                                int32_t t_begin, void *stream)
{
    if (T == 0 || B == 0) return DCLL_OK;
    if (!logits || !clout || T < 0 || B < 0 || N < 1) return fail(DCLL_ERR_INVALID, "dcll_argmax_vote: bad argument");
    if (vote && N > VOTE_MAXN) return fail(DCLL_ERR_UNSUPPORTED, "dcll_argmax_vote: vote supports at most 64 classes");
    if (T == 0 || B == 0) return DCLL_OK;
    hipStream_t st = (hipStream_t)stream;
    const long rows = (long)T * B;
    hipLaunchKernelGGL(k_argmax, dim3(nblk(rows, 256)), dim3(256), 0, st, logits, clout, rows, N);
    HIP_CHECK_LAUNCH("k_argmax");
    if (vote) {
        hipLaunchKernelGGL(k_vote, dim3(nblk(B, 64)), dim3(64), 0, st, clout, vote, T, B, N, t_begin);
        HIP_CHECK_LAUNCH("k_vote");
    }
    return DCLL_OK;
}

extern "C" int dcll_iq_encode(const float *iq, const float *thr_i, const float *thr_q, const dcll_iq_tail *tail,
                              int32_t *cells, int32_t B,
                              int32_t L, int32_t t0, int32_t T, int32_t w, int32_t h, void *stream)
{
    if (!iq || !thr_i || !thr_q || !cells || B < 0 || T < 0 || t0 < 0 || t0 + T > L || w < 1 || h < 1)
        return fail(DCLL_ERR_INVALID, "dcll_iq_encode: bad argument");
    if (tail && tail->tail_mask && (!tail->thr_i_tail || !tail->thr_q_tail))
        return fail(DCLL_ERR_INVALID, "dcll_iq_encode: tail mask without tail tables");
    if (T == 0 || B == 0) return DCLL_OK;
    hipLaunchKernelGGL(k_iq_encode, dim3(nblk((long)T * B, 256)), dim3(256), 0, (hipStream_t)stream, iq, thr_i, thr_q,
                       make_iq_tail(tail), cells, B, L, t0, T, w, h);
    HIP_CHECK_LAUNCH("k_iq_encode");
    return DCLL_OK;
}

extern "C" int dcll_unpack_spikes(const uint32_t *packed, float *dense, int64_t nwords, void *stream)
{
    if (nwords == 0) return DCLL_OK;
    if (!packed || !dense || nwords < 0) return fail(DCLL_ERR_INVALID, "dcll_unpack_spikes: bad argument");
    if (nwords == 0) return DCLL_OK;
    hipLaunchKernelGGL(k_unpack, dim3(nblk(nwords * 32, 256)), dim3(256), 0, (hipStream_t)stream, packed, dense, (long)nwords);
    HIP_CHECK_LAUNCH("k_unpack");
    return DCLL_OK;
}

extern "C" int dcll_pack_spikes(const float *dense, uint32_t *packed, int64_t nwords, void *stream)
{
    if (nwords == 0) return DCLL_OK;
    if (!packed || !dense || nwords < 0) return fail(DCLL_ERR_INVALID, "dcll_pack_spikes: bad argument");
    if (nwords == 0) return DCLL_OK;
    hipLaunchKernelGGL(k_pack, dim3(nblk(nwords * 32, 256)), dim3(256), 0, (hipStream_t)stream, dense, packed, (long)nwords);
    HIP_CHECK_LAUNCH("k_pack");
    return DCLL_OK;
}
```

Measured before the change: 21550.

## Rewrite time-paired c32 LIF kernel as output-stationary with prepacked weight fragments

Replaces the staged, slot-exchange time-paired conv-LIF kernel with an output-stationary version. Each wave owns two output rows, accumulates all 32 input channels itself, and streams prepacked weight fragments from a global workspace instead of holding them in registers. The eps1 trace images are double-buffered across four LDS images, which removes the per-stage slot writes and barriers of the old pipeline. The cost is an extra weight-packing kernel launch per call, a cached per-stream workspace, much larger LDS use that may limit occupancy, and global weight reloads inside the inner loop.

```diff
diff --git a/experiments/ablate_c32d.hip b/experiments/ablate_c32d.hip
--- a/experiments/ablate_c32d.hip
+++ b/experiments/ablate_c32d.hip
@@ -35,26 +35,26 @@
         for (int i = 0; i < n; ++i) dcll_launch_readout_direct(pv2, Wro, nullptr, ro, (long)T * B, 8192, 24, side);
     };
     if (tp) {
-        const char *names[3] = {"k_lif_seq_c32rp (row-paired)", "k_lif_seq_c32d (time-paired)", "k_lif_seq_c32d, chain phase only"};
-        for (int mode = 0; mode < 3; ++mode) {
-            for (int rep = 0; rep < 3 && mode < 2; ++rep) {
+        const char *names[2] = {"k_lif_seq_c32rp (row-paired)", "k_lif_seq_c32d (time-paired, output-stationary)"};
+        float *wfrag;
+        hipMalloc(&wfrag, OS_WFRAG_FLOATS * 4);
+        for (int mode = 0; mode < 2; ++mode) {
+            for (int rep = 0; rep < 3; ++rep) {
                 hipMemset(e0, 0, ns * 4); hipMemset(e1, 0, ns * 4); hipMemset(arp, 0, ns * 4);
                 hipEventRecord(a);
                 if (mode == 0)
                     hipLaunchKernelGGL((k_lif_seq_c32rp<true, 1, 0>), dim3(B), dim3(512), 0, 0, spk_in, dcll_wsrc{W, nullptr, nullptr}, bias, tau4, e0, e1, arp, spk_out, pv, (float *)nullptr, T, B, 0.65f, 1.0f);
-                else
-                    hipLaunchKernelGGL((k_lif_seq_c32d<true, 1, 0>), dim3(B), dim3(512), 0, 0, spk_in, dcll_wsrc{W, nullptr, nullptr}, bias, tau4, e0, e1, arp, spk_out, pv, (float *)nullptr, T, B, 0.65f, 1.0f);
+                else {
+                    hipLaunchKernelGGL(k_c32d_wfrag, dim3(OS_WFRAG_FLOATS / 256), dim3(256), 0, 0, dcll_wsrc{W, nullptr, nullptr}, wfrag);
+                    hipLaunchKernelGGL((k_lif_seq_c32d<true, 1>), dim3(B), dim3(512), 0, 0, spk_in, wfrag, bias, tau4, e0, e1, arp, spk_out, pv, (float *)nullptr, T, B, 0.65f, 1.0f);
+                }
                 hipEventRecord(b); hipEventSynchronize(b);
                 float ms; hipEventElapsedTime(&ms, a, b);
                 printf("%s B=%d T=%d: %.3f ms\n", names[mode], B, T, ms);
             }
+            if (mode == 1) continue;
             hipMemset(dbg, 0, 4096);
-            if (mode == 0)
-                hipLaunchKernelGGL((k_lif_seq_c32rp<true, 1, 1>), dim3(B), dim3(512), 0, 0, spk_in, dcll_wsrc{W, nullptr, nullptr}, bias, tau4, e0, e1, arp, spk_out, pv, (float *)dbg, T, B, 0.65f, 1.0f);
-            else if (mode == 1)
-                hipLaunchKernelGGL((k_lif_seq_c32d<true, 1, 1>), dim3(B), dim3(512), 0, 0, spk_in, dcll_wsrc{W, nullptr, nullptr}, bias, tau4, e0, e1, arp, spk_out, pv, (float *)dbg, T, B, 0.65f, 1.0f);
-            else
-                hipLaunchKernelGGL((k_lif_seq_c32d<true, 1, 9>), dim3(B), dim3(512), 0, 0, spk_in, dcll_wsrc{W, nullptr, nullptr}, bias, tau4, e0, e1, arp, spk_out, pv, (float *)dbg, T, B, 0.65f, 1.0f);
+            hipLaunchKernelGGL((k_lif_seq_c32rp<true, 1, 1>), dim3(B), dim3(512), 0, 0, spk_in, dcll_wsrc{W, nullptr, nullptr}, bias, tau4, e0, e1, arp, spk_out, pv, (float *)dbg, T, B, 0.65f, 1.0f);
             hipDeviceSynchronize();
             unsigned long long h4[64];
             hipMemcpy(h4, dbg, 512, hipMemcpyDeviceToHost);
diff --git a/snn_modulation_classification_amd/csrc/dcll_hip.hip b/snn_modulation_classification_amd/csrc/dcll_hip.hip
--- a/snn_modulation_classification_amd/csrc/dcll_hip.hip
+++ b/snn_modulation_classification_amd/csrc/dcll_hip.hip
@@ -1,4 +1,7 @@
 #include "dcll_internal.h"
+#include <map>
+#include <mutex>
+#include <utility>
 
 static thread_local char g_err[DCLL_ERR_LEN] = "";
 char *dcll_err_buf(void) { return g_err; }
@@ -1644,317 +1647,297 @@
     }
 }
 
-constexpr int TP_IMGP = IMG_FLOATS + 20;
-static_assert(TP_IMGP % 32 == 16 && TP_IMGP >= IMG_FLOATS, "image pitch");
 constexpr int TP_ROW_A[8] = {0, 1, 4, 6, 12, 13, 8, 10}, TP_ROW_B[8] = {3, 2, 5, 7, 15, 14, 9, 11};
-constexpr int tp_lo(int r) { return r - 3 < 0 ? 0 : r - 3; }
-constexpr int tp_hi(int r) { return r + 3 > 15 ? 15 : r + 3; }
-constexpr int tp_trace_m(int s) { return (s + 3) & 7; }
-constexpr bool tp_trace_next(int s) { return s >= 5; }
-constexpr bool tp_reads(int s, int rho) { return rho >= tp_lo(TP_ROW_A[s]) && rho <= tp_hi(TP_ROW_B[s]); }
-constexpr uint32_t tp_pack(const int (&r)[8])
-{
-    uint32_t p = 0;
-    for (int i = 0; i < 8; ++i) p |= (uint32_t)r[i] << (4 * i);
-    return p;
-}
-constexpr bool tp_schedule_ok()
-{
-    int seen = 0, mseen = 0;
-    for (int s = 0; s < 8; ++s) {
-        if (TP_ROW_A[s] >= TP_ROW_B[s]) return false;
-        if (tp_lo(TP_ROW_A[s]) > tp_lo(TP_ROW_B[s]) || tp_hi(TP_ROW_A[s]) > tp_hi(TP_ROW_B[s])) return false;
-        if (tp_lo(TP_ROW_B[s]) > tp_hi(TP_ROW_A[s]) + 1) return false;
-        seen |= (1 << TP_ROW_A[s]) | (1 << TP_ROW_B[s]);
-        const int s2 = (s + 2) & 7;
-        const int n = tp_hi(TP_ROW_A[s]) - tp_lo(TP_ROW_A[s]) + tp_hi(TP_ROW_B[s]) - tp_lo(TP_ROW_B[s]) + 2;
-        const int n2 = tp_hi(TP_ROW_A[s2]) - tp_lo(TP_ROW_A[s2]) + tp_hi(TP_ROW_B[s2]) - tp_lo(TP_ROW_B[s2]) + 2;
-        if (n + n2 != 25) return false;
-        const int m = tp_trace_m(s);
-        mseen |= 1 << m;
-        for (int rho = 2 * m; rho < 2 * m + 2; ++rho) {
-            if (tp_trace_next(s)) {
-                for (int u = s; u < 8; ++u) if (tp_reads(u, rho)) return false;
-            } else {
-                for (int u = 0; u < s; ++u) if (tp_reads(u, rho)) return false;
-                if (rho == tp_lo(TP_ROW_A[s])) return false;
-            }
-        }
-    }
-    return seen == 0xffff && mseen == 0xff;
-}
-static_assert(tp_schedule_ok(), "k_lif_seq_c32d: tile order / rolling trace schedule");
-
-template <bool REFRACTORY, int OUT, int DBG = 0>
-__global__ __launch_bounds__(512) void k_lif_seq_c32d(const uint32_t *__restrict__ spk_in, const dcll_wsrc W,
+constexpr int OS_CHF = 16 * ROWF;
+constexpr int OS_IMG = 32 * OS_CHF + 3;
+constexpr int OS_IMGP = 9744;
+constexpr int OS_LDS_FLOATS = 4 * OS_IMGP;
+constexpr int OS_WFRAG_FLOATS = 16 * 49 * 64;
+static_assert(OS_IMGP % 32 == 16 && OS_IMGP >= OS_IMG, "image pitch");
+static_assert(OS_LDS_FLOATS * sizeof(float) <= 160 * 1024, "k_lif_seq_c32d: four eps1 images in 160 KiB of LDS");
+constexpr bool os_tap(int r, int ky) { return r + ky - 3 >= 0 && r + ky - 3 <= 15; }
+constexpr int os_nky(int w)
+{
+    int n = 0;
+    for (int ky = 0; ky < 7; ++ky) n += os_tap(TP_ROW_A[w], ky) || os_tap(TP_ROW_B[w], ky);
+    return n;
+}
+constexpr int os_ky(int w, int i)
+{
+    for (int ky = 0; ky < 7; ++ky)
+        if ((os_tap(TP_ROW_A[w], ky) || os_tap(TP_ROW_B[w], ky)) && i-- == 0) return ky;
+    return -1;
+}
+constexpr int os_rows(int w)
+{
+    int n = 0;
+    for (int ky = 0; ky < 7; ++ky) n += (os_tap(TP_ROW_A[w], ky) ? 1 : 0) + (os_tap(TP_ROW_B[w], ky) ? 1 : 0);
+    return n;
+}
+constexpr bool os_trace_first(int w) { return os_rows(w) > 12; }
+constexpr int os_read_parity(int p) { return p & 1; }
+constexpr int os_write_parity(int p) { return (p + 1) & 1; }
+constexpr bool os_schedule_ok()
+{
+    int seen = 0, total = 0;
+    for (int w = 0; w < 8; ++w) {
+        if (seen & ((1 << TP_ROW_A[w]) | (1 << TP_ROW_B[w]))) return false;
+        seen |= (1 << TP_ROW_A[w]) | (1 << TP_ROW_B[w]);
+        total += os_rows(w);
+        if ((w & 2) == 0 && os_rows(w) + os_rows(w + 2) != 25) return false;
+        if ((w & 2) == 0 && os_trace_first(w) == os_trace_first(w + 2)) return false;
+    }
+    for (int p = 0; p < 4; ++p) {
+        if (os_write_parity(p) == os_read_parity(p) || os_write_parity(p) != os_read_parity(p + 1)) return false;
+        if (p > 0 && os_write_parity(p) != os_read_parity(p - 1)) return false;
+    }
+    return seen == 0xffff && total == 100;
+}
+static_assert(os_schedule_ok(), "k_lif_seq_c32d: row ownership / SIMD balance / image parity");
+
+__global__ __launch_bounds__(256) void k_c32d_wfrag(const dcll_wsrc W, float *__restrict__ wfrag)
+{
+    const int i = blockIdx.x * 256 + threadIdx.x;
+    if (i >= OS_WFRAG_FLOATS) return;
+    const int lane = i & 63, f = i >> 6, tap = f % 49, cp = f / 49, co = lane & 31, h = lane >> 5;
+    wfrag[i] = W.at(((long)co * 32 + 2 * cp + h) * 49 + tap, co);
+}
+
+template <bool REFRACTORY, int OUT>
+__global__ __launch_bounds__(512) void k_lif_seq_c32d(const uint32_t *__restrict__ spk_in, const float *__restrict__ wfrag,
                                                        const float *__restrict__ bias, const float *__restrict__ tau4,
                                                        float *__restrict__ eps0_g, float *__restrict__ eps1_g,
                                                        float *__restrict__ arp_g, uint32_t *__restrict__ spk_out,
                                                        float *__restrict__ pv_out, float *__restrict__ v_out, int T,
                                                        int B, float alpharp, float wrp)
 {
-    __shared__ __attribute__((aligned(16))) float lds[2 * TP_IMGP + (NWAVE * 2 + 1) * SLOT_FLOATS];
-    float *slots = lds + 2 * TP_IMGP;
-    float *sbias = slots + NWAVE * 2 * SLOT_FLOATS;
+    __shared__ __attribute__((aligned(16))) float lds[OS_LDS_FLOATS + 32];
+    float *sbias = lds + OS_LDS_FLOATS;
     const int tid = threadIdx.x, lane = tid & 63, h = lane >> 5, j = lane & 31, px = lane & 15, rb = (lane >> 4) & 1;
     const int wi = __builtin_amdgcn_readfirstlane(tid >> 6);
     const int w = (wi & 1) | ((wi & 4) >> 1) | ((wi & 2) << 1);
-    const int wq = w & 3, wpar = w >> 2;
     const long b = blockIdx.x;
     const int NP = T >> 1;
     __builtin_amdgcn_s_setprio(3);
 
-    for (int i = tid; i < 2 * TP_IMGP; i += 512) lds[i] = 0.0f;
-    for (int i = tid; i < SLOT_FLOATS; i += 512) sbias[i] = bias[(i & 3) + 8 * (i >> 8) + 4 * ((i >> 7) & 1)];
-
-    float wf[2][49];
-    load_wf_c32(W, j, w, h, wf);
-
-    float e0[8][2];
-    const int toff = (4 * w + h) * CHF + (rb + 3) * ROWF + px + 3;
-    float ta[2], tm[2], tas[2], ts[2];
-#pragma unroll
-    for (int e = 0; e < 2; ++e) {
-        ta[e] = tau4[0 * 32 + 4 * w + 2 * e + h]; tm[e] = tau4[1 * 32 + 4 * w + 2 * e + h];
-        tas[e] = tau4[2 * 32 + 4 * w + 2 * e + h]; ts[e] = tau4[3 * 32 + 4 * w + 2 * e + h];
-    }
-    const uint32_t *in_wave = spk_in + (b * 32 + 4 * w) * 8;
-    const long in_step = (long)B * 32 * 8;
-    auto in_mask = [&](long t, int e, int m) -> unsigned long long {
-        const uint32_t *ip = in_wave + t * in_step + 2 * e * 8 + m;
-        return (unsigned long long)ip[0] | ((unsigned long long)ip[8] << 32);
+    for (int i = tid; i < OS_LDS_FLOATS; i += 512) lds[i] = 0.0f;
+    if (tid < 32) sbias[tid] = bias[(tid & 3) + 8 * ((tid >> 2) & 3) + 4 * (tid >> 4)];
+
+    __syncthreads();
+
+    auto run = [&](auto WC) {
+        constexpr int W = decltype(WC)::value, RA = TP_ROW_A[W], RB = TP_ROW_B[W], NKY = os_nky(W);
+        constexpr int LO = RA - 3 < 0 ? 0 : RA - 3;
+        static_assert(RA < RB && ((RB + 3 > 15 ? 15 : RB + 3) - LO) * ROWF + 6 < 256, "B-fragment offsets within ds_read2_b32's range");
+        constexpr bool FIRST = os_trace_first(W);
+        float e0[8][2], e1[8][2];
+        float ta[2], tm[2], tas[2];
+        uint32_t tsb[2];
+    #pragma unroll
+        for (int e = 0; e < 2; ++e) {
+            ta[e] = tau4[0 * 32 + 4 * W + 2 * e + h]; tm[e] = tau4[1 * 32 + 4 * W + 2 * e + h];
+            tas[e] = tau4[2 * 32 + 4 * W + 2 * e + h]; tsb[e] = __float_as_uint(tau4[3 * 32 + 4 * W + 2 * e + h]);
+        }
+    #pragma unroll
+        for (int m = 0; m < 8; ++m)
+    #pragma unroll
+            for (int e = 0; e < 2; ++e) {
+                const long gidx = (b * 32 + 4 * W + 2 * e + h) * 256 + 32 * m + j;
+                e0[m][e] = eps0_g[gidx];
+                e1[m][e] = eps1_g[gidx];
+            }
+        const long in_step = (long)B * 32 * 8;
+        const uint32_t *in_lane = spk_in + (b * 32 + 4 * W + h) * 8;
+        uint32_t mw[2][2][8];
+        auto load_masks = [&](const int t2) {
+    #pragma unroll
+            for (int dt = 0; dt < 2; ++dt)
+    #pragma unroll
+                for (int e = 0; e < 2; ++e) {
+                    const uint4 *ip = (const uint4 *)(in_lane + (long)(t2 + dt) * in_step + 2 * e * 8);
+                    const uint4 q0 = ip[0], q1 = ip[1];
+                    mw[dt][e][0] = q0.x; mw[dt][e][1] = q0.y; mw[dt][e][2] = q0.z; mw[dt][e][3] = q0.w;
+                    mw[dt][e][4] = q1.x; mw[dt][e][5] = q1.y; mw[dt][e][6] = q1.z; mw[dt][e][7] = q1.w;
+                }
+        };
+        const int toff = (4 * W + h) * OS_CHF + rb * ROWF + px + 3;
+        auto trace = [&](const int par) {
+            float *dst = lds + 2 * par * OS_IMGP + toff;
+    #pragma unroll
+            for (int m = 0; m < 8; ++m)
+    #pragma unroll
+                for (int e = 0; e < 2; ++e)
+    #pragma unroll
+                    for (int dt = 0; dt < 2; ++dt) {
+                        const float a = __uint_as_float((uint32_t)__builtin_amdgcn_sbfe((int)mw[dt][e][m], j, 1) & tsb[e]);
+                        const float bb = tas[e] * e0[m][e];
+                        e0[m][e] = a + bb;
+                        const float cc = ta[e] * e1[m][e];
+                        const float dd = e0[m][e] * tm[e];
+                        e1[m][e] = cc + dd;
+                        dst[dt * OS_IMGP + e * 2 * OS_CHF + 2 * m * ROWF] = e1[m][e];
+                    }
+        };
+        load_masks(0);
+        trace(0);
+
+        const int bbase = h * OS_CHF + (j >> 4) * OS_IMGP + (j & 15);
+        const unsigned eoff = 4u * ((4 * h + rb) * 256 + px);
+        const unsigned soff = (unsigned)((lane >> 1) & 1) * ((unsigned)B * 1024u) +
+                              32u * (2 * ((lane >> 2) & 1) + 8 * ((lane >> 3) & 3) + 4 * (lane & 1));
+        const auto wrs = tile_rsrc(wfrag);
+        const unsigned wlane = 4u * lane;
+        const f32x4 *bvp = (const f32x4 *)(sbias + 16 * h);
+
+        float arpA[8], arpB[8];
+#pragma unroll
+        for (int m = 0; m < 8; ++m) {
+            const long aidx = (b * 32 + 2 * (m & 1) + 8 * (m >> 1) + 4 * h + rb) * 256 + px;
+            arpA[m] = REFRACTORY ? arp_g[aidx + RA * 16] : 0.0f;
+            arpB[m] = REFRACTORY ? arp_g[aidx + RB * 16] : 0.0f;
+        }
+        float wb[7][7];
+        static_for<0, NKY>([&](auto IC) {
+            constexpr int KY = os_ky(W, decltype(IC)::value);
+#pragma unroll
+            for (int kx = 0; kx < 7; ++kx)
+                wb[KY][kx] = __uint_as_float(__builtin_amdgcn_raw_buffer_load_b32(wrs, wlane, (KY * 7 + kx) * 256, 0));
+        });
+        if (FIRST && NP > 1) load_masks(2);
+        lds_barrier();
+
+        for (int p = 0; p < NP; ++p) {
+            if (FIRST && p + 1 < NP) {
+                trace(os_write_parity(p));
+            }
+            lds_cfloat *ib0 = (lds_cfloat *)(lds + bbase + 2 * os_read_parity(p) * OS_IMGP + LO * ROWF), *ib1 = ib0 + 2 * OS_CHF;
+            asm volatile("" : "+v"(ib0), "+v"(ib1));
+            f32x16 accA, accB;
+#pragma unroll
+            for (int c = 0; c < 4; ++c) {
+                const f32x4 q = bvp[c];
+                accA[4 * c + 0] = q[0]; accA[4 * c + 1] = q[1]; accA[4 * c + 2] = q[2]; accA[4 * c + 3] = q[3];
+            }
+            accB = accA;
+            float bqA[2][7], bqB[2][7];
+            auto fetch_b = [&](auto SETC, auto KYC, lds_cfloat *base) {
+                constexpr int SET = decltype(SETC)::value, KY = decltype(KYC)::value;
+#pragma unroll
+                for (int kx = 0; kx < 7; ++kx) {
+                    if (os_tap(RA, KY)) bqA[SET][kx] = base[(RA + KY - 3 - LO) * ROWF + kx];
+                    if (os_tap(RB, KY)) bqB[SET][kx] = base[(RB + KY - 3 - LO) * ROWF + kx];
+                }
+            };
+            fetch_b(std::integral_constant<int, 0>{}, std::integral_constant<int, os_ky(W, 0)>{}, ib0);
+#pragma nounroll
+            for (int c2 = 0; c2 < 8; ++c2) {
+                const unsigned wnext0 = (unsigned)(2 * c2 + 1) * (49u * 256u), wnext1 = (unsigned)((2 * c2 + 2) & 15) * (49u * 256u);
+                static_for<0, 2 * NKY>([&](auto RC) {
+                    constexpr int R = decltype(RC)::value, CPO = R / NKY, KY = os_ky(W, R % NKY);
+                    if constexpr (R + 1 == NKY) {
+                        ib0 += 4 * OS_CHF;
+                        asm volatile("" : "+v"(ib0));
+                    }
+                    if constexpr (R + 1 < 2 * NKY)
+                        fetch_b(std::integral_constant<int, (R + 1) & 1>{}, std::integral_constant<int, os_ky(W, (R + 1) % NKY)>{},
+                                (R + 1) / NKY ? ib1 : ib0);
+                    else if (c2 < 7)
+                        fetch_b(std::integral_constant<int, 0>{}, std::integral_constant<int, os_ky(W, 0)>{}, ib0);
+                    __builtin_amdgcn_sched_barrier(0);
+#pragma unroll
+                    for (int kx = 0; kx < 7; ++kx) {
+                        if (os_tap(RA, KY)) accA = __builtin_amdgcn_mfma_f32_32x32x2f32(wb[KY][kx], bqA[R & 1][kx], accA, 0, 0, 0);
+                        if (os_tap(RB, KY)) accB = __builtin_amdgcn_mfma_f32_32x32x2f32(wb[KY][kx], bqB[R & 1][kx], accB, 0, 0, 0);
+                    }
+                    __builtin_amdgcn_sched_barrier(0);
+                    const unsigned wo = CPO ? wnext1 : wnext0;
+#pragma unroll
+                    for (int kx = 0; kx < 7; ++kx)
+                        wb[KY][kx] = __uint_as_float(__builtin_amdgcn_raw_buffer_load_b32(wrs, wlane, wo + (KY * 7 + kx) * 256, 0));
+                    __builtin_amdgcn_sched_barrier(0);
+                });
+                ib1 += 4 * OS_CHF;
+                asm volatile("" : "+v"(ib1));
+            }
+            if (FIRST ? p + 2 < NP : p + 1 < NP) load_masks(FIRST ? 2 * p + 4 : 2 * p + 2);
+
+            const long ubase = ((long)(2 * p) * B + b) * 32 * 256, ustep = (long)B * 32 * 256;
+            auto epilogue = [&](f32x16 &acc, float (&arp)[8], auto ROWC) {
+                constexpr int ROW = decltype(ROWC)::value;
+                const auto prs0 = tile_rsrc(pv_out + ubase), prs1 = tile_rsrc(pv_out + ubase + ustep);
+                const auto vrs0 = tile_rsrc(v_out + ubase), vrs1 = tile_rsrc(v_out + ubase + ustep);
+                uint32_t pk = 0;
+#pragma unroll
+                for (int m = 0; m < 8; ++m) {
+                    const auto sw = __builtin_amdgcn_permlane16_swap(__float_as_uint(acc[2 * m]), __float_as_uint(acc[2 * m + 1]), false, false);
+                    float v0 = __uint_as_float(sw[0]), v1 = __uint_as_float(sw[1]);
+                    bool s0, s1;
+                    if (REFRACTORY) {
+                        v0 = refractory(v0, arp[m], alpharp, wrp, s0);
+                        v1 = refractory(v1, arp[m], alpharp, wrp, s1);
+                    } else {
+                        s0 = v0 > 0.0f; s1 = v1 > 0.0f;
+                    }
+                    const unsigned long long mk0 = __ballot(s0), mk1 = __ballot(s1);
+                    const int co = (2 * (m & 1) + 8 * (m >> 1)) * 1024 + ROW * 64;
+                    if (OUT & 1) {
+                        __builtin_amdgcn_raw_buffer_store_b32(__float_as_uint(sigmoidf_dev(v0)), prs0, eoff, co, 0);
+                        __builtin_amdgcn_raw_buffer_store_b32(__float_as_uint(sigmoidf_dev(v1)), prs1, eoff, co, 0);
+                    }
+                    if (OUT & 2) {
+                        __builtin_amdgcn_raw_buffer_store_b32(__float_as_uint(v0), vrs0, eoff, co, 0);
+                        __builtin_amdgcn_raw_buffer_store_b32(__float_as_uint(v1), vrs1, eoff, co, 0);
+                    }
+                    asm("s_nop 1\n\tv_writelane_b32 %0, %1, %2" : "+v"(pk) : "s"((uint32_t)mk0), "n"(4 * m + 0));
+                    asm("s_nop 1\n\tv_writelane_b32 %0, %1, %2" : "+v"(pk) : "s"((uint32_t)(mk0 >> 32)), "n"(4 * m + 1));
+                    asm("s_nop 1\n\tv_writelane_b32 %0, %1, %2" : "+v"(pk) : "s"((uint32_t)mk1), "n"(4 * m + 2));
+                    asm("s_nop 1\n\tv_writelane_b32 %0, %1, %2" : "+v"(pk) : "s"((uint32_t)(mk1 >> 32)), "n"(4 * m + 3));
+                }
+                if (spk_out && lane < 32) {
+                    const auto srs = tile_rsrc(spk_out + (ubase >> 5));
+                    __builtin_amdgcn_raw_buffer_store_b16((unsigned short)pk, srs, soff, 4 * (ROW >> 1) + 2 * (ROW & 1), 0);
+                    __builtin_amdgcn_raw_buffer_store_b16((unsigned short)(pk >> 16), srs, soff, 32 + 4 * (ROW >> 1) + 2 * (ROW & 1), 0);
+                }
+            };
+            epilogue(accA, arpA, std::integral_constant<int, RA>{});
+            epilogue(accB, arpB, std::integral_constant<int, RB>{});
+
+            if (!FIRST && p + 1 < NP) trace(os_write_parity(p));
+            lds_barrier();
+        }
+
+        if (REFRACTORY) {
+            int lo = 4 * h + rb;
+            asm volatile("" : "+v"(lo));
+#pragma unroll
+            for (int m = 0; m < 8; ++m) {
+                const long aidx = (b * 32 + 2 * (m & 1) + 8 * (m >> 1) + lo) * 256 + px;
+                arp_g[aidx + RA * 16] = arpA[m];
+                arp_g[aidx + RB * 16] = arpB[m];
+            }
+        }
+        int jo = j;
+        asm volatile("" : "+v"(jo));
+    #pragma unroll
+        for (int m = 0; m < 8; ++m)
+    #pragma unroll
+            for (int e = 0; e < 2; ++e) {
+                const long gidx = (b * 32 + 4 * W + 2 * e + h) * 256 + 32 * m + jo;
+                eps0_g[gidx] = e0[m][e];
+                eps1_g[gidx] = e1[m][e];
+            }
     };
-    __syncthreads();
-
-    static_for<0, 8>([&](auto SC) {
-        constexpr int S = decltype(SC)::value, M = tp_trace_m(S);
-#pragma unroll
-        for (int e = 0; e < 2; ++e) {
-            const long gidx = (b * 32 + 4 * w + 2 * e + h) * 256 + 32 * M + j;
-            e0[S][e] = eps0_g[gidx];
-            float e1 = eps1_g[gidx];
-            float *dst = lds + toff + e * 2 * CHF + 2 * M * ROWF;
-            trace_update((float)((in_mask(0, e, M) >> lane) & 1ull), ta[e], tm[e], tas[e], ts[e], e0[S][e], e1);
-            dst[0] = e1;
-            trace_update((float)((in_mask(1, e, M) >> lane) & 1ull), ta[e], tm[e], tas[e], ts[e], e0[S][e], e1);
-            dst[TP_IMGP] = e1;
-        }
-    });
-    const uint32_t rowpk = wpar ? tp_pack(TP_ROW_B) : tp_pack(TP_ROW_A);
-    const int ech = 8 * wq + 4 * h + 2 * rb;
-    float arp[8][2];
-#pragma unroll
-    for (int s = 0; s < 8; ++s) {
-        const int re = (rowpk >> (4 * ((s + w) & 7))) & 15;
-#pragma unroll
-        for (int k = 0; k < 2; ++k) arp[s][k] = REFRACTORY ? arp_g[(b * 32 + ech + k) * 256 + re * 16 + px] : 0.0f;
-    }
-
-    const int bbase = (4 * w + h) * CHF + (j >> 4) * TP_IMGP + (j & 15);
-    const int eslot = (7 * 2 + wpar) * SLOT_FLOATS + (wq * 64 + h * 32 + px) * 4 + 2 * rb;
-    const unsigned eoff = 4u * ((4 * h + 2 * rb) * 256 + px);
-    const unsigned soff = (unsigned)(px >> 1) * ((unsigned)B * 1024u) + 32u * (4 * h + 2 * rb + (px & 1));
-#pragma unroll
-    for (int s = 0; s < 8; ++s)
-#pragma unroll
-        for (int k = 0; k < 2; ++k) asm volatile("" ::"v"(arp[s][k]), "v"(e0[s][k]));
-#pragma unroll
-    for (int cp = 0; cp < 2; ++cp)
-#pragma unroll
-        for (int k = 0; k < 49; ++k) asm volatile("" ::"v"(wf[cp][k]));
-    __syncthreads();
-
-    unsigned long long dbg[4] = {0, 0, 0, 0}, dbg_t0 = 0;
-    if (DBG & 1) dbg_t0 = __builtin_amdgcn_s_memtime();
-    float sv[2] = {0.f, 0.f};
-    unsigned long long wm[2][2] = {{0, 0}, {0, 0}};
-    auto tracing = [&](const int q, const int s) {
-        const int P = q >> 3;
-        return !(DBG & 8) && q >= 0 && (tp_trace_next(s) ? P + 1 < NP : (P >= 1 && P < NP));
-    };
-    auto fetch_trace_inputs = [&](const int q, auto SC) {
-        constexpr int S = decltype(SC)::value, M = tp_trace_m(S);
-        if (tracing(q, S)) {
-            const long t2 = 2 * ((q >> 3) + (tp_trace_next(S) ? 1 : 0));
-#pragma unroll
-            for (int e = 0; e < 2; ++e) {
-                sv[e] = lds[TP_IMGP + toff + e * 2 * CHF + 2 * M * ROWF];
-                wm[e][0] = in_mask(t2, e, M);
-                wm[e][1] = in_mask(t2 + 1, e, M);
-            }
-        }
-    };
-    auto stage = [&](const int g, auto SC) {
-        constexpr int S = decltype(SC)::value, RA = TP_ROW_A[S], RB = TP_ROW_B[S];
-        constexpr int LO = tp_lo(RA), HI = tp_hi(RB), NRH = HI - LO + 1, NR = 2 * NRH;
-        unsigned long long st0 = 0, st1 = 0, st2 = 0, st3 = 0;
-        if (DBG & 1) st0 = __builtin_amdgcn_s_memtime();
-        const int q = g - w;
-        const bool active = q >= 0 && q < 8 * NP;
-        f32x16 accA, accB;
-        if (active) {
-            const float *inA = (w == 0) ? sbias : slots + ((w - 1) * 2) * SLOT_FLOATS;
-            const float *inB = (w == 0) ? sbias : slots + ((w - 1) * 2 + 1) * SLOT_FLOATS;
-            const f32x4 *spa = (const f32x4 *)inA + lane, *spb = (const f32x4 *)inB + lane;
-#pragma unroll
-            for (int c = 0; c < 4; ++c) {
-                f32x4 va = spa[c * 64], vb = spb[c * 64];
-                accA[4 * c + 0] = va[0]; accA[4 * c + 1] = va[1]; accA[4 * c + 2] = va[2]; accA[4 * c + 3] = va[3];
-                accB[4 * c + 0] = vb[0]; accB[4 * c + 1] = vb[1]; accB[4 * c + 2] = vb[2]; accB[4 * c + 3] = vb[3];
-            }
-        }
-        const int qe = g - 8;
-        const bool epi = !(DBG & 8) && qe >= 0 && qe < 8 * NP;
-        f32x2 v0 = {0.f, 0.f}, v1 = {0.f, 0.f};
-        if (epi) {
-            v0 = *(const f32x2 *)(slots + eslot);
-            v1 = *(const f32x2 *)(slots + eslot + 64);
-        }
-        lds_cfloat *ib0 = (lds_cfloat *)(lds + bbase + (LO + 3) * ROWF), *ib1 = (lds_cfloat *)(lds + bbase + (LO + 3) * ROWF + 2 * CHF);
-        asm volatile("" : "+v"(ib0), "+v"(ib1));
-        float bq[2][7];
-        if (active) {
-#pragma unroll
-            for (int kx = 0; kx < 7; ++kx) bq[0][kx] = ib0[kx];
-        }
-        if (tracing(q, S)) {
-            float *dst = lds + toff + 2 * tp_trace_m(S) * ROWF;
-#pragma unroll
-            for (int e = 0; e < 2; ++e) {
-                float e1 = sv[e];
-#pragma unroll
-                for (int dt = 0; dt < 2; ++dt) {
-                    float a;
-                    asm("v_cndmask_b32 %0, 0, %1, %2" : "=v"(a) : "v"(ts[e]), "s"(wm[e][dt]));
-                    const float bb = tas[e] * e0[S][e];
-                    e0[S][e] = a + bb;
-                    const float cc = ta[e] * e1;
-                    const float dd = e0[S][e] * tm[e];
-                    e1 = cc + dd;
-                    dst[e * 2 * CHF + dt * TP_IMGP] = e1;
-                }
-            }
-        }
-        if (epi) {
-            const int te = 2 * (qe >> 3);
-            const int re = (rowpk >> (4 * (g & 7))) & 15;
-            const long ubase = (((long)te * B + b) * 32 + 8 * wq) * 256, ustep = (long)B * 32 * 256;
-            float vv[2][2];
-            unsigned long long mk[2][2];
-#pragma unroll
-            for (int k = 0; k < 2; ++k) {
-                bool s0, s1;
-                if (REFRACTORY) {
-                    vv[k][0] = refractory(v0[k], arp[S][k], alpharp, wrp, s0);
-                    vv[k][1] = refractory(v1[k], arp[S][k], alpharp, wrp, s1);
-                } else {
-                    vv[k][0] = v0[k]; vv[k][1] = v1[k];
-                    s0 = v0[k] > 0.0f; s1 = v1[k] > 0.0f;
-                }
-                mk[k][0] = __ballot(s0); mk[k][1] = __ballot(s1);
-            }
-#pragma unroll
-            for (int dt = 0; dt < 2; ++dt) {
-                const auto prs = tile_rsrc(pv_out + ubase + dt * ustep), vrs = tile_rsrc(v_out + ubase + dt * ustep);
-#pragma unroll
-                for (int k = 0; k < 2; ++k) {
-                    if (OUT & 1) __builtin_amdgcn_raw_buffer_store_b32(__float_as_uint(sigmoidf_dev(vv[k][dt])), prs, eoff + 4u * (k * 256), re * 64, 0);
-                    if (OUT & 2) __builtin_amdgcn_raw_buffer_store_b32(__float_as_uint(vv[k][dt]), vrs, eoff + 4u * (k * 256), re * 64, 0);
-                }
-            }
-            if (spk_out) {
-                uint32_t myword = 0;
-#pragma unroll
-                for (int dt = 0; dt < 2; ++dt)
-#pragma unroll
-                    for (int k = 0; k < 2; ++k) {
-                        const uint32_t mine = h ? (uint32_t)(mk[k][dt] >> 32) : (uint32_t)mk[k][dt];
-                        myword = (px == k + 2 * dt) ? mine : myword;
-                    }
-                myword >>= 16 * rb;
-                if (px < 4)
-                    __builtin_amdgcn_raw_buffer_store_b16((unsigned short)myword, tile_rsrc(spk_out + (ubase >> 5)), soff, 4 * (re >> 1) + 2 * (re & 1), 0);
-            }
-        }
-        if (DBG & 1) { asm volatile("s_waitcnt lgkmcnt(0)" ::: "memory"); st1 = __builtin_amdgcn_s_memtime(); }
-        lds_barrier();
-        if (DBG & 1) st2 = __builtin_amdgcn_s_memtime();
-        fetch_trace_inputs(q + 1, std::integral_constant<int, (S + 1) & 7>{});
-        if (active) {
-#pragma unroll
-            for (int r = 0; r < NR; ++r) {
-                const int cp = r / NRH, rho = LO + r % NRH;
-                if (r + 1 < NR) {
-                    const int cpn = (r + 1) / NRH, rhon = (r + 1) % NRH;
-#pragma unroll
-                    for (int kx = 0; kx < 7; ++kx) bq[(r + 1) & 1][kx] = (cpn ? ib1 : ib0)[rhon * ROWF + kx];
-                }
-                __builtin_amdgcn_sched_barrier(0);
-#pragma unroll
-                for (int kx = 0; kx < 7; ++kx) {
-                    if (rho >= tp_lo(RA) && rho <= tp_hi(RA))
-                        accA = __builtin_amdgcn_mfma_f32_32x32x2f32(wf[cp][(rho - RA + 3) * 7 + kx], bq[r & 1][kx], accA, 0, 0, 0);
-                    if (rho >= tp_lo(RB) && rho <= tp_hi(RB))
-                        accB = __builtin_amdgcn_mfma_f32_32x32x2f32(wf[cp][(rho - RB + 3) * 7 + kx], bq[r & 1][kx], accB, 0, 0, 0);
-                }
-                __builtin_amdgcn_sched_barrier(0);
-                if (cp == 1 && rho == tp_hi(RA)) {
-                    f32x4 *dpa = (f32x4 *)(slots + (w * 2) * SLOT_FLOATS) + lane;
-#pragma unroll
-                    for (int c = 0; c < 4; ++c)
-                        dpa[c * 64] = f32x4{accA[4 * c + 0], accA[4 * c + 1], accA[4 * c + 2], accA[4 * c + 3]};
-                    __builtin_amdgcn_sched_barrier(0);
-                }
-            }
-            f32x4 *dp = (f32x4 *)(slots + (w * 2 + 1) * SLOT_FLOATS) + lane;
-#pragma unroll
-            for (int c = 0; c < 4; ++c)
-                dp[c * 64] = f32x4{accB[4 * c + 0], accB[4 * c + 1], accB[4 * c + 2], accB[4 * c + 3]};
-        }
-        if (DBG & 1) { asm volatile("s_waitcnt lgkmcnt(0)" ::: "memory"); st3 = __builtin_amdgcn_s_memtime(); }
-        lds_barrier();
-        if (DBG & 1) {
-            const unsigned long long st4 = __builtin_amdgcn_s_memtime();
-            dbg[0] += st1 - st0; dbg[1] += st2 - st1; dbg[2] += st3 - st2; dbg[3] += st4 - st3;
-        }
-    };
-
-    const int nstage = 8 * NP + 8;
-    for (int g = 0; g < nstage; ++g) {
-        switch ((g - w) & 7) {
-        case 0: stage(g, std::integral_constant<int, 0>{}); break;
-        case 1: stage(g, std::integral_constant<int, 1>{}); break;
-        case 2: stage(g, std::integral_constant<int, 2>{}); break;
-        case 3: stage(g, std::integral_constant<int, 3>{}); break;
-        case 4: stage(g, std::integral_constant<int, 4>{}); break;
-        case 5: stage(g, std::integral_constant<int, 5>{}); break;
-        case 6: stage(g, std::integral_constant<int, 6>{}); break;
-        default: stage(g, std::integral_constant<int, 7>{}); break;
-        }
-    }
-
-    if ((DBG & 1) && lane == 0 && b == 0) {
-        unsigned long long *dp = (unsigned long long *)v_out + w * 8;
-        dp[0] = __builtin_amdgcn_s_memtime() - dbg_t0;
-        dp[1] = dbg[0]; dp[2] = dbg[1]; dp[3] = dbg[2]; dp[4] = dbg[3];
-    }
-    static_for<0, 8>([&](auto SC) {
-        constexpr int S = decltype(SC)::value, M = tp_trace_m(S);
-#pragma unroll
-        for (int e = 0; e < 2; ++e) {
-            const long gidx = (b * 32 + 4 * w + 2 * e + h) * 256 + 32 * M + j;
-            eps0_g[gidx] = e0[S][e];
-            eps1_g[gidx] = lds[TP_IMGP + toff + e * 2 * CHF + 2 * M * ROWF];
-        }
-    });
-    if (REFRACTORY) {
-#pragma unroll
-        for (int s = 0; s < 8; ++s) {
-            const int re = (rowpk >> (4 * ((s + w) & 7))) & 15;
-#pragma unroll
-            for (int k = 0; k < 2; ++k) arp_g[(b * 32 + ech + k) * 256 + re * 16 + px] = arp[s][k];
-        }
-    }
+    switch (w) {
+    case 0: run(std::integral_constant<int, 0>{}); break;
+    case 1: run(std::integral_constant<int, 1>{}); break;
+    case 2: run(std::integral_constant<int, 2>{}); break;
+    case 3: run(std::integral_constant<int, 3>{}); break;
+    case 4: run(std::integral_constant<int, 4>{}); break;
+    case 5: run(std::integral_constant<int, 5>{}); break;
+    case 6: run(std::integral_constant<int, 6>{}); break;
+    default: run(std::integral_constant<int, 7>{}); break;
+    }
+
 }
 
 __global__ void k_permute_readout(const float *__restrict__ Wt, float *__restrict__ Wp, int N)
@@ -3354,6 +3337,36 @@
 #undef DCLL_LAUNCH_C32
 }
 
+static int c32d_workspace(hipStream_t st, float **out)
+{
+    static std::mutex mu;
+    static std::map<std::pair<int, hipStream_t>, float *> ws;
+    int dev = 0;
+    if (hipGetDevice(&dev) != hipSuccess) {
+        (void)hipGetLastError();
+        return fail(DCLL_ERR_LAUNCH, "hipGetDevice failed", "dcll_conv_lif_sequence");
+    }
+    std::lock_guard<std::mutex> guard(mu);
+    const auto key = std::make_pair(dev, st);
+    const auto it = ws.find(key);
+    if (it != ws.end()) {
+        *out = it->second;
+        return DCLL_OK;
+    }
+    void *p = nullptr;
+    hipStreamCaptureMode mode = hipStreamCaptureModeRelaxed;
+    (void)hipThreadExchangeStreamCaptureMode(&mode);
+    const hipError_t e = hipMalloc(&p, OS_WFRAG_FLOATS * sizeof(float));
+    (void)hipThreadExchangeStreamCaptureMode(&mode);
+    if (e != hipSuccess || !p) {
+        (void)hipGetLastError();
+        return fail(DCLL_ERR_LAUNCH, "no memory for the weight workspace of k_lif_seq_c32d", "dcll_conv_lif_sequence");
+    }
+    ws[key] = (float *)p;
+    *out = (float *)p;
+    return DCLL_OK;
+}
+
 static int dcll_conv_lif_sequence_run(const dcll_conv_desc *d, const uint32_t *spk_in, dcll_wsrc W, const float *b,
                                       const float *tau4, float *eps0, float *eps1, float *arp, uint32_t *spk_out,
                                       float *pv_out, float *v_out, const float *ro_Wp, const float *ro_b,
@@ -3371,7 +3384,7 @@
     if (n_ro == 0 && T >= DCLL_C32D_MIN_T) {
         const bool tp = (T & 1) == 0;
 #define DCLL_LAUNCH_C32D(K, R, O)                                                                                       \
-    hipLaunchKernelGGL((K<R, O>), dim3(B), dim3(512), 0, st, spk_in, W, b, tau4, eps0, eps1, arp, spk_out, pv_out,      \
+    hipLaunchKernelGGL((K<R, O>), dim3(B), dim3(512), 0, st, spk_in, WSRC, b, tau4, eps0, eps1, arp, spk_out, pv_out,   \
                        v_out, T, B, d->alpharp, d->wrp)
 #define DCLL_LAUNCH_C32D_O(K, R)                                                                                        \
     switch (out) {                                                                                                     \
@@ -3381,9 +3394,19 @@
     default: DCLL_LAUNCH_C32D(K, R, 3); break;                                                                         \
     }
         if (tp) {
+            float *WSRC = nullptr;
+            const int rc = c32d_workspace(st, &WSRC);
+            if (rc) return rc;
+            hipLaunchKernelGGL(k_c32d_wfrag, dim3(OS_WFRAG_FLOATS / 256), dim3(256), 0, st, W, WSRC);
+            const hipError_t eh = hipGetLastError();
+            if (eh != hipSuccess) {
+                snprintf(dcll_err_buf(), DCLL_ERR_LEN, "k_c32d_wfrag: %s", hipGetErrorString(eh));
+                return DCLL_ERR_LAUNCH;
+            }
             if (d->refractory) { DCLL_LAUNCH_C32D_O(k_lif_seq_c32d, true) } else { DCLL_LAUNCH_C32D_O(k_lif_seq_c32d, false) }
             HIP_CHECK_LAUNCH("k_lif_seq_c32d");
         } else {
+            const dcll_wsrc WSRC = W;
             if (d->refractory) { DCLL_LAUNCH_C32D_O(k_lif_seq_c32rp, true) } else { DCLL_LAUNCH_C32D_O(k_lif_seq_c32rp, false) }
             HIP_CHECK_LAUNCH("k_lif_seq_c32rp");
         }
```

After: 22010 (median of 6 runs). 1.02x the previous value.
